# klasmodin/quflow

Measured on AMD Instinct MI355X. Metric: isospectral timesteps/sec at N=1024 (1 GPU) + ensemble steps/sec at 1/2/4/8 GPUs, higher is better.
Workload: dtype f64

## Files before the change

### include/quflow_hip.h

```cpp
#ifndef QUFLOW_HIP_H
#define QUFLOW_HIP_H

#ifdef __cplusplus
extern "C" {
#endif

#define QF_OK 0
#define QF_ERR_INVALID 1
#define QF_ERR_NO_DEVICE 2
#define QF_ERR_HIP 3
#define QF_ERR_STATE 4
#define QF_ERR_CALLBACK 5
#define QF_ERR_UNSUPPORTED 6
#define QF_ERR_NONFINITE 7
#define QF_ERR_NOCONVERGE 8

#define QF_VERSION 100

typedef struct qf_ctx qf_ctx;

int qf_version(void);
const char *qf_last_error(void);
int qf_device_count(void);

// ... 83 lines not shown
    int (*forcing)(void *user, const void *P, const void *Whalf, void *F, double time);
    int (*strang)(void *user, double h, void *W);
    int (*callback)(void *user, const void *W, const void *dW2);
    int hamiltonian_takes_time, forcing_takes_time;
    int has_time;
    double time;
    int skewh;
    int solve_skewh;
    const double *strang_table;
    unsigned long long strang_key;
    int magnetic;
    int states_p;
} qf_isomp_hooks;
int qf_isomp_hooked(qf_ctx *ctx, void *states_host, int k, double dt, int steps, double tol, int minit, int maxit,
                    int compsum, int reinitialize, const qf_isomp_hooks *hooks, qf_isomp_stats *stats_out);
int qf_isomp_forced(qf_ctx *ctx, double dt, int steps, double tol, int minit, int maxit, int reinitialize,
                    const double *strang_table, unsigned long long strang_key, qf_isomp_stats *stats_out);
int qf_erk_hooked(qf_ctx *ctx, void *W_host, int method, double dt, int steps, const qf_isomp_hooks *hooks);
int qf_erk_states_hooked(qf_ctx *ctx, void *states_host, int k, int method, double dt, int steps, const qf_isomp_hooks *hooks);

int qf_basis_upload(qf_ctx *ctx, const double *basis_host, long long count);
int qf_basis_compute(qf_ctx *ctx);
int qf_basis_download(qf_ctx *ctx, double *basis_host, long long count);
int qf_basis_stream(qf_ctx *ctx, long long slab_bytes);
int qf_basis_slab_plan(int N, int Nmax, long long slab_bytes, int *first_block, int capacity);
int qf_shr2mat(qf_ctx *ctx, const double *omega_host, long long n_omega, void *W_host);
int qf_mat2shr(qf_ctx *ctx, const void *W_host, double *omega_host, long long n_omega);
int qf_shc2mat(qf_ctx *ctx, const void *omega_host, void *W_host);
int qf_mat2shc(qf_ctx *ctx, const void *W_host, void *omega_host);
int qf_shr2fun(qf_ctx *ctx, const double *omega_host, long long n_omega, int L, int berezin, double *f_host);
int qf_shc2fun(qf_ctx *ctx, const void *omega_host, long long n_omega, int L, int berezin, int isreal, void *f_host);
int qf_fun2shc(qf_ctx *ctx, const void *f_host, int L, int isreal, void *omega_host);
int qf_fun2shr(qf_ctx *ctx, const void *f_host, int L, int isreal, double *omega_host);

int qf_diagnostics(qf_ctx *ctx, double *energy_euler, double *enstrophy);
int qf_isomp_diag(qf_ctx *ctx, double dt, int steps, double tol, int minit, int maxit, int compsum,
                  int reinitialize, qf_isomp_stats *stats, double *energy_euler, double *enstrophy);
int qf_norm_inf_W(qf_ctx *ctx, double *out);

typedef struct qf_eigh_stats {
    int sweeps;
    long long rotations;
    double off;
} qf_eigh_stats;
int qf_eigh(qf_ctx *ctx, const void *H_host, double *lambda_host, void *V_host, qf_eigh_stats *stats);
int qf_eigh_skew(qf_ctx *ctx, const void *W_host, double *lambda_host, void *V_host, qf_eigh_stats *stats);
int qf_eigh_state(qf_ctx *ctx, double *lambda_host, qf_eigh_stats *stats);
int qf_scale_decomposition(qf_ctx *ctx, const void *W_host, const void *P_host, void *Ws_host, void *Wr_host);

int qf_so3_exp_plan(int N, const double xi[3], int *squarings, int *degree);
int qf_so3_exp(qf_ctx *ctx, const double xi[3], void *R_host);
int qf_so3_exp_times(qf_ctx *ctx, double *taylor_ms, double *squarings_ms);
int qf_rotate(qf_ctx *ctx, const double xi[3], const void *W_host, void *out_host);
int qf_grad(qf_ctx *ctx, const void *P_host, void *dP_host);

#define QF_KERNEL_POISSON 0
#define QF_KERNEL_GEMM1 1
#define QF_KERNEL_GEMM2 2
#define QF_KERNEL_NORM 3
#define QF_KERNEL_UPDATE 4
#define QF_KERNEL_SLICE 5
#define QF_KERNEL_COUNT 6

int qf_profile_enable(qf_ctx *ctx, int mask);
int qf_profile_reset(qf_ctx *ctx);
int qf_profile_read(qf_ctx *ctx, int kernel_id, long long *launches, double *total_ms);
int qf_profile_stride(qf_ctx *ctx, int stride);
int qf_profile_seen(qf_ctx *ctx, int kernel_id, long long *seen);
int qf_device_info(int device, char *buf, int n);
int qf_plan_describe(qf_ctx *ctx, char *buf, int n);
int qf_timer_start(qf_ctx *ctx);
int qf_timer_stop(qf_ctx *ctx, double *elapsed_ms);

#define QF_BUF_W 0
#define QF_BUF_DW 1
#define QF_BUF_WHALF 2
#define QF_BUF_PHALF 3
#define QF_BUF_PW 4
int qf_download_buffer(qf_ctx *ctx, int which, void *host);
int qf_debug_guard_check(long long *allocations, long long *damaged, char *first, int n);
int qf_debug_modulus(qf_ctx *ctx, int n, const double *er_host, const double *ei_host, double *out_modulus_host,
                     double *out_sqrt_host);
int qf_zgemm(qf_ctx *ctx, const void *A_host, const void *B_host, void *C_host);
int qf_commutator(qf_ctx *ctx, const void *W_host, const void *P_host, void *C_host, int skewherm);
int qf_zgemm_i8(qf_ctx *ctx, const void *A_host, const void *B_host, void *C_host);
int qf_fixedpoint_products(qf_ctx *ctx, const void *Phalf_host, const void *Whalf_host, const void *W_host,
                           const void *dW_old_host, int variant, void *dW_new_host, void *Whalf_new_host,
                           double *rowsum_host);

int qf_c64_laplacian_table(qf_ctx *ctx, int bc, float *lap_host);
int qf_c64_solve_poisson(qf_ctx *ctx, const void *W_host, void *P_host, int skewh);
int qf_c64_solve_tridiagonal(qf_ctx *ctx, const float *lap_host, const void *W_host, void *P_host, int skewh);
int qf_c64_laplace(qf_ctx *ctx, const void *P_host, void *W_host);
int qf_c64_upload_W(qf_ctx *ctx, const void *W_host);
int qf_c64_download_W(qf_ctx *ctx, void *W_host);
int qf_c64_isomp(qf_ctx *ctx, double dt, int steps, double tol, int minit, int maxit, int compsum, int reinitialize,
                 qf_isomp_stats *stats_out);
int qf_c64_isomp_continue(qf_ctx *ctx, double dt, int steps, double tol, int minit, int maxit, int compsum, int reinitialize,
                          qf_isomp_stats *stats_out);
int qf_c64_diagnostics(qf_ctx *ctx, double *energy_euler, double *enstrophy);
int qf_cgemm(qf_ctx *ctx, const void *A_host, const void *B_host, void *C_host);
int qf_c64_fixedpoint_products(qf_ctx *ctx, const void *Phalf_host, const void *Whalf_host, const void *W_host,
                               const void *dW_old_host, void *dW_new_host, void *Whalf_new_host, double *rowsum_host);
int qf_c64_fixedpoint_products_tri(qf_ctx *ctx, const void *Phalf_host, const void *Whalf_host, const void *W_host,
                                   const void *dW_old_host, void *dW_new_host, void *Whalf_new_host, double *rowsum_host);

#define QF_COMM_ID_BYTES 128
typedef struct qf_comm qf_comm;
int qf_comm_unique_id(void *id128);
int qf_comm_create(qf_comm **out, int device, int nranks, int rank, const void *id128);
int qf_comm_allgather_f64(qf_comm *comm, const double *send_host, int count, double *recv_host);
int qf_comm_barrier(qf_comm *comm);
int qf_comm_destroy(qf_comm *comm);

#ifdef __cplusplus
}
#endif
#endif
```

### quflow_amd/_lib.py

```python
import ctypes
import os

_HERE = os.path.dirname(os.path.abspath(__file__))
LIB_PATH = os.environ.get("QUFLOW_HIP_LIB") or os.path.join(_HERE, "libquflow_hip.so")

QF_OK = 0
QF_ERR_NONFINITE = 7
QF_ERR_NOCONVERGE = 8
ERR_NAMES = {1: "QF_ERR_INVALID", 2: "QF_ERR_NO_DEVICE", 3: "QF_ERR_HIP", 4: "QF_ERR_STATE", 5: "QF_ERR_CALLBACK",
             6: "QF_ERR_UNSUPPORTED", 7: "QF_ERR_NONFINITE", 8: "QF_ERR_NOCONVERGE"}

KERNEL_IDS = {"poisson": 0, "gemm1": 1, "gemm2": 2, "norm": 3, "update": 4, "slice": 5}
ERK_METHODS = {"euler": 0, "heun": 1, "rk4": 2}
BUFFER_IDS = {"W": 0, "dW": 1, "Whalf": 2, "Phalf": 3, "PW": 4}


class QuflowHipError(RuntimeError):
    pass


HAMILTONIAN_CB = ctypes.CFUNCTYPE(ctypes.c_int, ctypes.c_void_p, ctypes.c_void_p, ctypes.c_void_p, ctypes.c_double)
FORCING_CB = ctypes.CFUNCTYPE(ctypes.c_int, ctypes.c_void_p, ctypes.c_void_p, ctypes.c_void_p, ctypes.c_void_p, ctypes.c_double)
STRANG_CB = ctypes.CFUNCTYPE(ctypes.c_int, ctypes.c_void_p, ctypes.c_double, ctypes.c_void_p)
CALLBACK_CB = ctypes.CFUNCTYPE(ctypes.c_int, ctypes.c_void_p, ctypes.c_void_p, ctypes.c_void_p)
# ... 63 lines not shown
    "qf_comm_unique_id": (ctypes.c_int, [_vp]),
    "qf_comm_create": (ctypes.c_int, [ctypes.POINTER(_vp), ctypes.c_int, ctypes.c_int, ctypes.c_int, _vp]),
    "qf_comm_allgather_f64": (ctypes.c_int, [_vp, _vp, ctypes.c_int, _vp]),
    "qf_comm_barrier": (ctypes.c_int, [_vp]),
    "qf_comm_destroy": (ctypes.c_int, [_vp]),
    "qf_upload_W": (ctypes.c_int, [_vp, _vp]),
    "qf_download_W": (ctypes.c_int, [_vp, _vp]),
    "qf_isomp": (ctypes.c_int, [_vp, ctypes.c_double, ctypes.c_int, ctypes.c_double, ctypes.c_int,
                                ctypes.c_int, ctypes.c_int, ctypes.c_int, ctypes.POINTER(IsompStats)]),
    "qf_isomp_diag": (ctypes.c_int, [_vp, ctypes.c_double, ctypes.c_int, ctypes.c_double, ctypes.c_int,
                                     ctypes.c_int, ctypes.c_int, ctypes.c_int, ctypes.POINTER(IsompStats),
                                     ctypes.POINTER(ctypes.c_double), ctypes.POINTER(ctypes.c_double)]),
    "qf_isomp_continue": (ctypes.c_int, [_vp, ctypes.c_double, ctypes.c_int, ctypes.c_double, ctypes.c_int,
                                         ctypes.c_int, ctypes.c_int, ctypes.c_int, ctypes.POINTER(IsompStats)]),
    "qf_isomp_multi": (ctypes.c_int, [ctypes.POINTER(_vp), ctypes.c_int, ctypes.c_double, ctypes.c_int, ctypes.c_double,
                                      ctypes.c_int, ctypes.c_int, ctypes.POINTER(IsompStats)]),
    "qf_c64_isomp_multi": (ctypes.c_int, [ctypes.POINTER(_vp), ctypes.c_int, ctypes.c_double, ctypes.c_int, ctypes.c_double,
                                          ctypes.c_int, ctypes.c_int, ctypes.POINTER(IsompStats)]),
    "qf_erk": (ctypes.c_int, [_vp, ctypes.c_int, ctypes.c_double, ctypes.c_int, ctypes.c_int]),
    "qf_erk_states": (ctypes.c_int, [_vp, _vp, ctypes.c_int, ctypes.c_int, ctypes.c_double, ctypes.c_int, ctypes.c_int]),
    "qf_isomp_simple_hooked": (ctypes.c_int, [_vp, ctypes.c_double, ctypes.c_int, ctypes.POINTER(IsompHooks)]),
    "qf_isomp_quasinewton_hooked": (ctypes.c_int, [_vp, ctypes.c_double, ctypes.c_int, ctypes.c_double, ctypes.c_int,
                                                   ctypes.POINTER(IsompStats), ctypes.POINTER(IsompHooks)]),
    "qf_isomp_simple": (ctypes.c_int, [_vp, ctypes.c_double, ctypes.c_int]),
    "qf_isomp_quasinewton": (ctypes.c_int, [_vp, ctypes.c_double, ctypes.c_int, ctypes.c_double, ctypes.c_int,
                                            ctypes.POINTER(IsompStats)]),
    "qf_isomp_states": (ctypes.c_int, [_vp, _vp, ctypes.c_int, ctypes.c_double, ctypes.c_int, ctypes.c_double,
                                       ctypes.c_int, ctypes.c_int, ctypes.c_int, ctypes.c_int,
                                       ctypes.POINTER(IsompStats)]),
    "qf_states_upload": (ctypes.c_int, [_vp, _vp, ctypes.c_int]),
    "qf_states_download": (ctypes.c_int, [_vp, _vp, ctypes.c_int]),
    "qf_states_advance": (ctypes.c_int, [_vp, ctypes.c_double, ctypes.c_int, ctypes.c_double, ctypes.c_int, ctypes.c_int,
                                         ctypes.c_int, ctypes.c_int, ctypes.POINTER(IsompStats)]),
    "qf_states_advance_diag": (ctypes.c_int, [_vp, ctypes.c_double, ctypes.c_int, ctypes.c_double, ctypes.c_int, ctypes.c_int,
                                              ctypes.c_int, ctypes.c_int, ctypes.POINTER(IsompStats), _dp]),
    "qf_states_select": (ctypes.c_int, [_vp, ctypes.c_int]),
    "qf_states_store": (ctypes.c_int, [_vp, ctypes.c_int]),
    "qf_mhd_diagnostics": (ctypes.c_int, [_vp, _dp]),
    "qf_states_inner": (ctypes.c_int, [_vp, _dp]),
    "qf_isomp_hooked": (ctypes.c_int, [_vp, _vp, ctypes.c_int, ctypes.c_double, ctypes.c_int, ctypes.c_double, ctypes.c_int,
                                       ctypes.c_int, ctypes.c_int, ctypes.c_int, ctypes.POINTER(IsompHooks),
                                       ctypes.POINTER(IsompStats)]),
    "qf_erk_hooked": (ctypes.c_int, [_vp, _vp, ctypes.c_int, ctypes.c_double, ctypes.c_int, ctypes.POINTER(IsompHooks)]),
    "qf_erk_states_hooked": (ctypes.c_int, [_vp, _vp, ctypes.c_int, ctypes.c_int, ctypes.c_double, ctypes.c_int,
                                            ctypes.POINTER(IsompHooks)]),
    "qf_basis_upload": (ctypes.c_int, [_vp, _vp, ctypes.c_longlong]),
    "qf_basis_compute": (ctypes.c_int, [_vp]),
    "qf_basis_download": (ctypes.c_int, [_vp, _vp, ctypes.c_longlong]),
    "qf_basis_stream": (ctypes.c_int, [_vp, ctypes.c_longlong]),
    "qf_basis_slab_plan": (ctypes.c_int, [ctypes.c_int, ctypes.c_int, ctypes.c_longlong, ctypes.POINTER(ctypes.c_int),
                                          ctypes.c_int]),
    "qf_shr2mat": (ctypes.c_int, [_vp, _vp, ctypes.c_longlong, _vp]),
    "qf_mat2shr": (ctypes.c_int, [_vp, _vp, _vp, ctypes.c_longlong]),
    "qf_shc2mat": (ctypes.c_int, [_vp, _vp, _vp]),
    "qf_mat2shc": (ctypes.c_int, [_vp, _vp, _vp]),
    "qf_shr2fun": (ctypes.c_int, [_vp, _vp, ctypes.c_longlong, ctypes.c_int, ctypes.c_int, _vp]),
    "qf_shc2fun": (ctypes.c_int, [_vp, _vp, ctypes.c_longlong, ctypes.c_int, ctypes.c_int, ctypes.c_int, _vp]),
    "qf_fun2shc": (ctypes.c_int, [_vp, _vp, ctypes.c_int, ctypes.c_int, _vp]),
    "qf_fun2shr": (ctypes.c_int, [_vp, _vp, ctypes.c_int, ctypes.c_int, _vp]),
    "qf_diagnostics": (ctypes.c_int, [_vp, _dp, _dp]),
    "qf_norm_inf_W": (ctypes.c_int, [_vp, _dp]),
    "qf_eigh": (ctypes.c_int, [_vp, _vp, _vp, _vp, ctypes.POINTER(EighStats)]),
    "qf_eigh_skew": (ctypes.c_int, [_vp, _vp, _vp, _vp, ctypes.POINTER(EighStats)]),
    "qf_eigh_state": (ctypes.c_int, [_vp, _vp, ctypes.POINTER(EighStats)]),
    "qf_scale_decomposition": (ctypes.c_int, [_vp, _vp, _vp, _vp, _vp]),
    "qf_so3_exp_plan": (ctypes.c_int, [ctypes.c_int, _dp, ctypes.POINTER(ctypes.c_int), ctypes.POINTER(ctypes.c_int)]),
    "qf_so3_exp": (ctypes.c_int, [_vp, _dp, _vp]),
    "qf_so3_exp_times": (ctypes.c_int, [_vp, _dp, _dp]),
    "qf_rotate": (ctypes.c_int, [_vp, _dp, _vp, _vp]),
    "qf_grad": (ctypes.c_int, [_vp, _vp, _vp]),
    "qf_profile_enable": (ctypes.c_int, [_vp, ctypes.c_int]),
    "qf_profile_reset": (ctypes.c_int, [_vp]),
    "qf_profile_read": (ctypes.c_int, [_vp, ctypes.c_int, ctypes.POINTER(ctypes.c_longlong), _dp]),
    "qf_plan_describe": (ctypes.c_int, [_vp, ctypes.c_char_p, ctypes.c_int]),
    "qf_device_info": (ctypes.c_int, [ctypes.c_int, ctypes.c_char_p, ctypes.c_int]),
    "qf_debug_modulus": (ctypes.c_int, [_vp, ctypes.c_int, _dp, _dp, _dp, _dp]),
    "qf_profile_stride": (ctypes.c_int, [_vp, ctypes.c_int]),
    "qf_profile_seen": (ctypes.c_int, [_vp, ctypes.c_int, ctypes.POINTER(ctypes.c_longlong)]),
    "qf_timer_start": (ctypes.c_int, [_vp]),
    "qf_timer_stop": (ctypes.c_int, [_vp, _dp]),
    "qf_download_buffer": (ctypes.c_int, [_vp, ctypes.c_int, _vp]),
    "qf_debug_guard_check": (ctypes.c_int, [ctypes.POINTER(ctypes.c_longlong), ctypes.POINTER(ctypes.c_longlong), ctypes.c_char_p, ctypes.c_int]),
    "qf_zgemm": (ctypes.c_int, [_vp, _vp, _vp, _vp]),
    "qf_commutator": (ctypes.c_int, [_vp, _vp, _vp, _vp, ctypes.c_int]),
    "qf_zgemm_i8": (ctypes.c_int, [_vp, _vp, _vp, _vp]),
    "qf_fixedpoint_products": (ctypes.c_int, [_vp, _vp, _vp, _vp, _vp, ctypes.c_int, _vp, _vp, _vp]),
    "qf_c64_laplacian_table": (ctypes.c_int, [_vp, ctypes.c_int, _vp]),
    "qf_c64_solve_poisson": (ctypes.c_int, [_vp, _vp, _vp, ctypes.c_int]),
    "qf_c64_laplace": (ctypes.c_int, [_vp, _vp, _vp]),
    "qf_c64_solve_tridiagonal": (ctypes.c_int, [_vp, _vp, _vp, _vp, ctypes.c_int]),
    "qf_c64_upload_W": (ctypes.c_int, [_vp, _vp]),
    "qf_c64_download_W": (ctypes.c_int, [_vp, _vp]),
    "qf_c64_isomp": (ctypes.c_int, [_vp, ctypes.c_double, ctypes.c_int, ctypes.c_double, ctypes.c_int,
                                    ctypes.c_int, ctypes.c_int, ctypes.c_int, ctypes.POINTER(IsompStats)]),
    "qf_c64_isomp_continue": (ctypes.c_int, [_vp, ctypes.c_double, ctypes.c_int, ctypes.c_double, ctypes.c_int,
                                             ctypes.c_int, ctypes.c_int, ctypes.c_int, ctypes.POINTER(IsompStats)]),
    "qf_c64_diagnostics": (ctypes.c_int, [_vp, _dp, _dp]),
    "qf_cgemm": (ctypes.c_int, [_vp, _vp, _vp, _vp]),
    "qf_c64_fixedpoint_products": (ctypes.c_int, [_vp, _vp, _vp, _vp, _vp, _vp, _vp, _vp]),
    "qf_c64_fixedpoint_products_tri": (ctypes.c_int, [_vp, _vp, _vp, _vp, _vp, _vp, _vp, _vp]),
}

_lib = None


def load():
    global _lib
    if _lib is None:
        if not os.path.exists(LIB_PATH):
            raise QuflowHipError(
                "libquflow_hip.so is not built (%s). Run `python -c 'import __graft_entry__ as g; g.build()'` "
                "or `make -C quflow_amd/csrc`. There is no CPU fallback." % LIB_PATH)
        lib = ctypes.CDLL(LIB_PATH)
        for name, (res, args) in SIGNATURES.items():
            fn = getattr(lib, name)
            fn.restype = res
            fn.argtypes = args
        _lib = lib
    return _lib


def check(rc):
    if rc == 7:
        raise ValueError("array must not contain infs or NaNs")
    if rc != QF_OK:
        msg = load().qf_last_error()
        raise QuflowHipError("%s: %s" % (ERR_NAMES.get(rc, "error %d" % rc),
                                         msg.decode("utf-8", "replace") if msg else ""))


def check_eigh(rc):
    if rc != QF_OK:
        msg = load().qf_last_error()
        raise QuflowHipError("%s: %s" % (ERR_NAMES.get(rc, "error %d" % rc),
                                         msg.decode("utf-8", "replace") if msg else ""))


def device_count():
    return load().qf_device_count()


def device_info(device):
    import json
    lib = load()
    n = lib.qf_device_info(int(device), None, 0)
    if n < 0:
        check(-n)
    buf = ctypes.create_string_buffer(n + 1)
    lib.qf_device_info(int(device), buf, n + 1)
    return json.loads(buf.value.decode())
```

### quflow_amd/csrc/api_context.hip

```cpp
#include <cmath>
#include <cstdarg>
#include <cstdio>
#include <cstdlib>
#include <cstring>
#include <limits>
#include <chrono>

#include "qf_api.h"

static thread_local char g_err[512] = "";

void qf_set_error(const char *fmt, ...)
{
    va_list ap;
    va_start(ap, fmt);
    vsnprintf(g_err, sizeof(g_err), fmt, ap);
    va_end(ap);
}

extern "C" {

int qf_version(void) { return QF_VERSION; }

int qf_device_info(int device, char *buf, int n)
// ... 33 lines not shown
    if (!ctx || (n > 0 && !buf) || n < 0) {
        qf_set_error("qf_plan_describe: bad arguments");
        return -QF_ERR_INVALID;
    }
    static const char *const role[QF_KERNEL_COUNT] = {"laplacian_inverse", "first_product", "second_product", "residual_norm",
                                                      "step_update", "slicing"};
    std::string out = "{\"N\": " + std::to_string(ctx->N);
    for (int r = 0; r < QF_KERNEL_COUNT; ++r) {
        out += ", \"";
        out += role[r];
        out += "\": ";
        out += ctx->plan[r].text[0] ? ctx->plan[r].text : "null";
    }
    if (ctx->ham_table || ctx->ham_offset_on) {
        char h[160];
        if (ctx->ham_table) snprintf(h, sizeof(h), ", \"hamiltonian\": {\"table_key\": %llu, \"offset\": %s}", ctx->ham_key, ctx->ham_offset_on ? "true" : "false");
        else snprintf(h, sizeof(h), ", \"hamiltonian\": {\"table_key\": null, \"offset\": true}");
        out += h;
    } else {
        out += ", \"hamiltonian\": \"poisson\"";
    }
    out += "}";
    if (n > 0) {
        const size_t m = out.size() < (size_t)(n - 1) ? out.size() : (size_t)(n - 1);
        memcpy(buf, out.data(), m);
        buf[m] = 0;
    }
    return (int)out.size();
}

const char *qf_last_error(void) { return g_err; }

int qf_device_count(void)
{
    int n = 0;
    if (hipGetDeviceCount(&n) != hipSuccess) return 0;
    return n;
}

double qf_hbar(int N) { return 2.0 / std::sqrt((double)N * (double)N - 1.0); }

int qf_ctx_create(int N, int device, qf_ctx **out)
{
    if (!out) {
        qf_set_error("qf_ctx_create: out is null");
        return QF_ERR_INVALID;
    }
    *out = nullptr;
    if (N < 2 || N > 8192) {
        qf_set_error("qf_ctx_create: N=%d out of range [2, 8192]", N);
        return QF_ERR_INVALID;
    }
    int ndev = qf_device_count();
    if (ndev <= 0) {
        qf_set_error("qf_ctx_create: no HIP device visible (this library has no CPU fallback)");
        return QF_ERR_NO_DEVICE;
    }
    if (device < 0 || device >= ndev) {
        qf_set_error("qf_ctx_create: device %d out of range (0..%d)", device, ndev - 1);
        return QF_ERR_NO_DEVICE;
    }
    QF_HIP(hipSetDevice(device));
    qf_ctx *ctx = new qf_ctx();
    ctx->N = N;
    ctx->device = device;
    if (const char *g = getenv("QUFLOW_HIP_GEMM")) {
        ctx->gemm_i8_allowed = (g[0] == 'i');
        if (g[0] == 'i' && strstr(g, "x6")) ctx->oz_digits = 6;
        if (g[0] == 'i' && strstr(g, "x65")) ctx->oz_digits2 = 5;
        if (g[0] == 'i' && strchr(g, 'h')) ctx->gemm_i8_hybrid = true;
        if (g[0] == 'i' && strchr(g, 'f') && !ctx->gemm_i8_hybrid) ctx->gemm_i8_first = true;
        if (g[0] == 'a') {
            ctx->gemm_i8_allowed = true;
            ctx->oz_digits = 6;
            ctx->oz_digits2 = 5;
            ctx->gemm_i8_min_n = 1024;
        }
    }
    if (const char *g = getenv("QUFLOW_HIP_GEMM2")) ctx->gemm_tri_allowed = !(g[0] == 'f');
    if (const char *g = getenv("QUFLOW_HIP_FUSED")) ctx->fused_allowed = !(g[0] == '0');
    if (const char *g = getenv("QUFLOW_HIP_I8_MIN_N")) ctx->gemm_i8_min_n = atoi(g);
    if (const char *g = getenv("QUFLOW_HIP_TRI_MIN_N")) ctx->gemm_tri_min_n = atoi(g);
    if (const char *g = getenv("QUFLOW_HIP_DEFER")) ctx->defer_allowed = !(g[0] == '0');
    if (getenv("QUFLOW_HIP_DEBUG"))
        if (const char *g = getenv("QUFLOW_HIP_DEBUG_DROP_FLAG")) ctx->debug_drop = atoi(g);
    if (const char *g = getenv("QUFLOW_HIP_FACTOR_CACHE_MB")) ctx->factor_budget_bytes = (size_t)(atoi(g) > 0 ? atoi(g) : 1) << 20;
    const size_t NN = (size_t)N * N;
    const size_t mbytes = NN * sizeof(cplx);
    int rc = QF_OK;
    auto fail = [&](int code) {
        qf_ctx_destroy(ctx);
        return code;
    };
#define QF_CREATE_HIP(call)                                                                   \
    do {                                                                                      \
        hipError_t _e = (call);                                                               \
        if (_e != hipSuccess) {                                                               \
            qf_set_error("%s failed: %s", #call, hipGetErrorString(_e));                     \
            return fail(QF_ERR_HIP);                                                          \
        }                                                                                     \
    } while (0)
    QF_CREATE_HIP(hipStreamCreateWithFlags(&ctx->stream, hipStreamNonBlocking));
    cplx **mats[] = {&ctx->W, &ctx->dW[0], &ctx->dW[1], &ctx->Whalf, &ctx->Phalf, &ctx->PW, &ctx->stage};
    for (cplx **m : mats) {
        QF_CREATE_HIP(hipMalloc((void **)m, mbytes));
        QF_CREATE_HIP(hipMemsetAsync(*m, 0, mbytes, ctx->stream));
    }
    QF_CREATE_HIP(hipMalloc((void **)&ctx->lap, 2 * NN * sizeof(double)));
    ctx->rowpart_tiles = qf_gemm_tiles_n(N);
    {
        const int slots32 = (N + 31) / 32;
        QF_CREATE_HIP(hipMalloc((void **)&ctx->rowpart, (size_t)(ctx->rowpart_tiles > slots32 ? ctx->rowpart_tiles : slots32) * N * sizeof(double)));
    }
    QF_CREATE_HIP(hipMalloc((void **)&ctx->rowsum, (size_t)N * sizeof(double)));
    QF_CREATE_HIP(hipMalloc((void **)&ctx->scalars, 4096 * sizeof(double)));
    QF_CREATE_HIP(hipHostMalloc((void **)&ctx->host_scalars, 64 * sizeof(double), hipHostMallocDefault));
    QF_CREATE_HIP(hipMalloc((void **)&ctx->state, sizeof(qf_dev_state)));
    QF_CREATE_HIP(hipMemsetAsync(ctx->state, 0, sizeof(qf_dev_state), ctx->stream));
    QF_CREATE_HIP(hipMalloc((void **)&ctx->ticket, 704 * sizeof(unsigned)));
    QF_CREATE_HIP(hipMemsetAsync(ctx->ticket, 0, 704 * sizeof(unsigned), ctx->stream));
    QF_CREATE_HIP(hipHostMalloc((void **)&ctx->host_rec, sizeof(qf_host_record), hipHostMallocCoherent));
    memset(ctx->host_rec, 0, sizeof(qf_host_record));
    {
        hipDeviceProp_t prop;
        QF_CREATE_HIP(hipGetDeviceProperties(&prop, device));
        ctx->num_cus = prop.multiProcessorCount;
        if (N % 64 == 0 && ctx->num_cus > 0) {
            ctx->sk_slots = ctx->num_cus;
            QF_CREATE_HIP(hipMalloc((void **)&ctx->sk_partial, (size_t)ctx->sk_slots * 64 * 64 * sizeof(cplx)));
            QF_CREATE_HIP(hipMalloc((void **)&ctx->sk_flags, (size_t)(ctx->sk_slots + 16) * sizeof(unsigned)));
            QF_CREATE_HIP(hipMemsetAsync(ctx->sk_flags, 0, (size_t)(ctx->sk_slots + 16) * sizeof(unsigned), ctx->stream));
        }
    }
    QF_CREATE_HIP(hipEventCreate(&ctx->timer_start));
    QF_CREATE_HIP(hipEventCreate(&ctx->timer_stop));
#undef QF_CREATE_HIP
    if ((rc = alloc_factors(ctx, &ctx->poisson)) != QF_OK) return fail(rc);
    if ((rc = qf_launch_lap_table(ctx, 1, ctx->lap)) != QF_OK) return fail(rc);
    if ((rc = qf_launch_build_factors(ctx, ctx->lap, ctx->poisson)) != QF_OK) return fail(rc);
    if (hipStreamSynchronize(ctx->stream) != hipSuccess) {
        qf_set_error("qf_ctx_create: table construction failed");
        return fail(QF_ERR_HIP);
    }
    *out = ctx;
    return QF_OK;
}

int qf_ctx_destroy(qf_ctx *ctx)
{
    if (!ctx) return QF_OK;
    (void)hipSetDevice(ctx->device);
    if (ctx->stream) (void)hipStreamSynchronize(ctx->stream);
    void *ptrs[] = {ctx->W, ctx->dW[0], ctx->dW[1], ctx->Whalf, ctx->Phalf, ctx->PW, ctx->kahan_c, ctx->stage,
                    ctx->lap, ctx->lap_user, ctx->poisson.tab, ctx->ham.tab, ctx->ham_offset, ctx->forcing_f0, ctx->stoch.basis, ctx->stoch.omega,
                    ctx->stoch.stage, ctx->stoch.sigma, ctx->rowpart, ctx->rowsum,
                    ctx->t32_partial, ctx->t32_arrive, ctx->W2, ctx->Whalf2, ctx->ns_inv, ctx->ns_tmp, ctx->multi_rowpart, ctx->scalars, ctx->sk_partial, ctx->sk_flags, ctx->basis, ctx->sh_stage, ctx->sh_omega, ctx->slab};
    for (void *p : ptrs)
        if (p) (void)hipFree(p);
    void *sht[] = {ctx->sht.omega, ctx->sht.tab, ctx->sht.col, ctx->sht.At, ctx->sht.tw, ctx->sht.f, ctx->sht.H, ctx->sht.Q};
    for (void *p : sht)
        if (p) (void)hipFree(p);
    void *eigh[] = {ctx->eigh.H, ctx->eigh.G, ctx->eigh.V, ctx->eigh.ray, ctx->eigh.sig, ctx->eigh.perm, ctx->eigh.word};
    for (void *p : eigh)
        if (p) (void)hipFree(p);
    void *geom[] = {ctx->geom.R[0], ctx->geom.R[1], ctx->geom.grad};
    for (void *p : geom)
// ... 228 lines not shown
```

### quflow_amd/csrc/api_isomp.hip

```cpp
#include <cmath>
#include <cstdarg>
#include <cstdio>
#include <cstdlib>
#include <cstring>
#include <limits>
#include <chrono>
#include <type_traits>
#include <utility>

#include "qf_api.h"

namespace {

#ifndef QF_RUN_AHEAD
#define QF_RUN_AHEAD 3
#endif

template <class S> constexpr bool is_c64 = std::is_same<S, qf_c64>::value;

template <class S> S *ws(qf_ctx *ctx)
{
    if constexpr (is_c64<S>) return ctx->c64;
    else return ctx;
}
// ... 99 lines not shown
        if (f->w_skew_known) {
            QF_TRY(qf_c64_tri_alloc(ctx));
            f->tri = true;
        }
    }
    return QF_OK;
}

bool triangle_product(const qf_ctx *ctx) { return (ctx->gemm_tri || ctx->gemm_tri32) && (!ctx->gemm_i8 || ctx->gemm_i8_first); }
bool triangle_product(const qf_c64 *f) { return f->tri; }

template <class S> int begin_increment(qf_ctx *ctx, S *w, bool carry)
{
    const size_t mbytes = (size_t)ctx->N * ctx->N * sizeof(*w->W);
    if (carry) {
        if (w->dw_cur != 0)
            QF_HIP(hipMemcpyAsync(w->dW[0], w->dW[w->dw_cur], mbytes, hipMemcpyDeviceToDevice, ctx->stream));
        QF_TRY(qf_launch_lincomb(ctx, 1, w->W, 1, w->dW[0], 0, w->Whalf));
    } else {
        QF_HIP(hipMemsetAsync(w->dW[0], 0, mbytes, ctx->stream));
        QF_HIP(hipMemcpyAsync(w->Whalf, w->W, mbytes, hipMemcpyDeviceToDevice, ctx->stream));
    }
    return QF_OK;
}

template <class S> int enqueue_iterations(qf_ctx *ctx, int step, int first, int count, double vareps)
{
    S *w = ws<S>(ctx);
    for (int i = first; i < first + count; ++i) {
        qf_guard g;
        g.state = ctx->state;
        g.step = step;
        g.iter = i;
        {
            prof_scope p(ctx, QF_KERNEL_POISSON);
            QF_TRY(launch_solve(ctx, w->Whalf, w->Phalf, vareps, g));
        }
        {
            prof_scope p(ctx, QF_KERNEL_GEMM1);
            QF_TRY(launch_gemm(ctx, w->Phalf, w->Whalf, w->PW, nullptr, g));
        }
        {
            prof_scope p(ctx, QF_KERNEL_GEMM2);
            const auto ep = epilogue_of(w, false);
            QF_TRY(launch_gemm(ctx, w->PW, w->Phalf, nullptr, &ep, g));
        }
        {
            prof_scope p(ctx, QF_KERNEL_NORM);
            QF_TRY(qf_launch_norm_decide(ctx, w->rowpart, is_c64<S> ? w->rowpart_tiles : qf_rowpart_slots(ctx), g));
        }
    }
    return QF_OK;
}

qf_decide deferred_decision(qf_ctx *ctx)
{
    qf_decide d;
    d.rowpart = ctx->rowpart;
    d.slots = ctx->gemm_tri32 ? (ctx->N + 31) / 32 : ctx->N / 64;
    d.state_rw = ctx->state;
    d.rec = ctx->host_rec;
    d.ticket = ctx->ticket + 402;
    return d;
}

template <class S> int enqueue_iterations_fused(qf_ctx *ctx, int step, int first, int count, double vareps, bool last_step)
{
    S *w = ws<S>(ctx);
    const bool defer = !is_c64<S> && ctx->defer;
    const qf_decide dec = defer ? deferred_decision(ctx) : qf_decide();
    for (int i = first; i < first + count; ++i) {
        qf_guard g;
        g.state = ctx->state;
        g.step = step;
        g.iter = i;
        g.alt = w->Whalf2;
        {
            prof_scope p(ctx, QF_KERNEL_POISSON);
            if constexpr (is_c64<S>) QF_TRY(launch_solve(ctx, w->Whalf, w->Phalf, vareps, g));
            else QF_TRY(launch_solve(ctx, w->Whalf, w->Phalf, vareps, g, defer ? &dec : nullptr));
        }
        {
            prof_scope p(ctx, QF_KERNEL_GEMM1);
            QF_TRY(launch_gemm(ctx, w->Phalf, w->Whalf, w->PW, nullptr, g));
        }
        {
            prof_scope p(ctx, QF_KERNEL_GEMM2);
            const auto ep = epilogue_of(w, true);
            g.alt = nullptr;
            if constexpr (is_c64<S>) {
                if (w->tri) QF_TRY(qf_launch_cgemm_tri(ctx, w->PW, w->Phalf, &ep, g));
                else QF_TRY(qf_launch_cgemm(ctx, w->PW, w->Phalf, nullptr, &ep, g));
            } else {
                QF_TRY(qf_launch_zgemm(ctx, w->PW, w->Phalf, nullptr, &ep, g));
            }
        }
    }
    if (defer && last_step && count > 0) QF_TRY(qf_launch_decide(ctx, dec));
    return QF_OK;
}

int enqueue_iterations_fused_i8(qf_ctx *ctx, int step, int first, int count, double vareps)
{
    for (int i = first; i < first + count; ++i) {
        qf_guard g;
        g.state = ctx->state;
        g.step = step;
        g.iter = i;
        g.alt = ctx->Whalf2;
        {
            prof_scope p(ctx, QF_KERNEL_POISSON);
            QF_TRY(qf_launch_hamiltonian(ctx, ctx->Whalf, ctx->Phalf, vareps, g));
        }
        if (ctx->gemm_i8_hybrid) {
            {
                prof_scope p(ctx, QF_KERNEL_GEMM1);
                QF_TRY(qf_launch_zgemm(ctx, ctx->Phalf, ctx->Whalf, ctx->PW, nullptr, g));
            }
            g.alt = nullptr;
            {
                prof_scope p(ctx, QF_KERNEL_SLICE);
                qf_oz_jobs jobs;
                jobs.n = 2;
                jobs.j[0].X = ctx->PW;
                jobs.j[0].planes = ctx->oz_planes[3];
                jobs.j[0].scale = ctx->oz_scale[3];
                jobs.j[1].X = ctx->Phalf;
                jobs.j[1].planes = ctx->oz_planes[0];
                jobs.j[1].scale = ctx->oz_scale[0];
                QF_TRY(qf_launch_oz_slice(ctx, jobs, g));
            }
            {
                prof_scope p(ctx, QF_KERNEL_GEMM2);
                const qf_epilogue ep = epilogue_of(ctx, true);
                QF_TRY(qf_launch_oz_gemm(ctx, ctx->oz_planes[3], ctx->oz_scale[3], ctx->oz_planes[0], ctx->oz_scale[0], nullptr,
                                         &ep, g));
            }
            continue;
        }
        g.alt = nullptr;
        {
            prof_scope p(ctx, QF_KERNEL_SLICE);
            qf_oz_jobs jobs;
            jobs.n = 2;
            jobs.j[0].X = ctx->Phalf;
            jobs.j[0].planes = ctx->oz_planes[0];
            jobs.j[0].scale = ctx->oz_scale[0];
            jobs.j[1].X = ctx->Whalf;
            jobs.j[1].X_alt = ctx->Whalf2;
            jobs.j[1].planes = ctx->oz_planes[2];
            jobs.j[1].scale = ctx->oz_scale[2];
            jobs.diag = ctx->oz_diag;
            QF_TRY(qf_launch_oz_slice(ctx, jobs, g));
        }
        {
            prof_scope p(ctx, QF_KERNEL_GEMM1);
            QF_TRY(qf_launch_oz_gemm(ctx, ctx->oz_planes[0], ctx->oz_scale[0], ctx->oz_planes[2], ctx->oz_scale[2],
                                     ctx->PW, nullptr, g, 0, 0, ctx->oz_diag));
        }
        if (ctx->gemm_i8_first) {
            prof_scope p(ctx, QF_KERNEL_GEMM2);
            const qf_epilogue ep = epilogue_of(ctx, true);
            QF_TRY(qf_launch_zgemm(ctx, ctx->PW, ctx->Phalf, nullptr, &ep, g));
            continue;
        }
        {
            prof_scope p(ctx, QF_KERNEL_SLICE);
            qf_oz_jobs jobs;
            jobs.n = 1;
            jobs.j[0].X = ctx->PW;
            jobs.j[0].planes = ctx->oz_planes[3];
// ... 126 lines not shown
        sched_yield();
        return;
    }
#if defined(__x86_64__)
    __builtin_ia32_pause();
#endif
}

template <class S> int run_fused(qf_ctx *ctx, int steps, int minit, int maxit, double vareps)
{
    fused_run<S> run;
    run.begin(ctx, steps, minit, maxit, vareps);
    while (!run.done()) {
        QF_TRY(run.pump());
        poll_relax();
    }
    ctx->pred_iters = run.pred;
    return QF_OK;
}

template <class S> int enqueue_step_end(qf_ctx *ctx, int step, int compsum, int reinitialize)
{
    S *w = ws<S>(ctx);
    qf_guard g;
    g.state = ctx->state;
    g.step = step;
    prof_scope p(ctx, QF_KERNEL_UPDATE);
    return qf_launch_update(ctx, w->PW, w->W, w->dW[0], w->dW[1], w->Whalf, compsum ? w->kahan_c : nullptr, reinitialize, g);
}

int wait_for_advance(qf_ctx *ctx, unsigned long long seq)
{
    volatile qf_host_record *rec = ctx->host_rec;
    unsigned long long spins = 0;
    while (__atomic_load_n(&rec->seq, __ATOMIC_ACQUIRE) < seq) {
        if (++spins > (1ull << 22)) {
            const unsigned long long before = __atomic_load_n(&rec->seq, __ATOMIC_ACQUIRE);
            const hipError_t q = hipStreamQuery(ctx->stream);
            QF_HIP(hipStreamSynchronize(ctx->stream));
            if (getenv("QUFLOW_HIP_DEBUG"))
                fprintf(stderr, "[quflow_hip] wait_for_advance: spin limit; want seq %llu, saw %llu before sync (stream %s), %llu after; step_index %d incomplete %d\n",
                        seq, before, q == hipSuccess ? "idle" : "busy", (unsigned long long)rec->seq, rec->step_index, rec->incomplete);
            if (__atomic_load_n(&rec->seq, __ATOMIC_ACQUIRE) < seq) {
                qf_set_error("qf_isomp: device progress record stuck at %llu (< %llu)",
                             (unsigned long long)rec->seq, seq);
                return QF_ERR_STATE;
            }
            break;
        }
#if defined(__x86_64__)
        __builtin_ia32_pause();
#endif
    }
    return QF_OK;
}

int reset_after_abort(qf_ctx *ctx)
{
    if (!ctx->needs_reset) return QF_OK;
    QF_HIP(hipMemsetAsync(ctx->ticket, 0, 704 * sizeof(unsigned), ctx->stream));
    if (ctx->sk_flags) QF_HIP(hipMemsetAsync(ctx->sk_flags + (ctx->sk_slots > 0 ? ctx->sk_slots : ctx->num_cus), 0, 16 * sizeof(unsigned), ctx->stream));
    if (ctx->t32_arrive) {
        const size_t nt = (size_t)(ctx->N + 31) / 32;
        QF_HIP(hipMemsetAsync(ctx->t32_arrive, 0, nt * (nt + 1) / 2 * sizeof(unsigned), ctx->stream));
    }
    if (ctx->c64 && ctx->c64->tri_arrive)
        QF_HIP(hipMemsetAsync(ctx->c64->tri_arrive, 0, ctx->c64->tri_arrive_count * sizeof(unsigned), ctx->stream));
    ctx->needs_reset = false;
    return QF_OK;
}

template <class S> int fused_enter(qf_ctx *ctx, double dt, double tol, int minit, int maxit, bool carry)
{
    S *w = ws<S>(ctx);
    const size_t mbytes = (size_t)ctx->N * ctx->N * sizeof(*w->W);
    const bool tol_on_device = tol < 0;
    const double tol_factor = tol_on_device ? mach_eps<S>(true) * dt / qf_hbar(ctx->N) : 0.0;
    QF_TRY(reset_after_abort(ctx));
    if constexpr (is_c64<S>) {
        QF_TRY(select_second_product_c64(ctx));
    } else {
        QF_TRY(select_second_product(ctx));
        ctx->defer = ctx->defer_allowed && !ctx->gemm_i8 && ctx->gemm_tri32 && ctx->N <= 512;
    }
    w->increment_is_zero = !carry;
    w->increment_valid = true;
    volatile qf_host_record *rec = ctx->host_rec;
    rec->progress = 0ull;
    rec->step_index = 0;
    rec->fault = 0;
    rec->nonfinite = 0;
    __atomic_thread_fence(__ATOMIC_SEQ_CST);
    if (is_c64<S> || carry) {
        if (tol_on_device) QF_TRY(qf_launch_norm_inf(ctx, w->W, ctx->scalars));
        QF_TRY(begin_increment(ctx, w, carry));
        QF_TRY(qf_launch_state_init(ctx, tol, minit, maxit, tol_on_device ? ctx->scalars : nullptr, tol_factor));
    } else {
        QF_TRY(qf_launch_call_begin(ctx, tol, minit, maxit, tol_on_device ? 1 : 0, tol_factor));
    }
    if (!w->W2) QF_HIP(hipMalloc((void **)&w->W2, mbytes));
    if (!w->Whalf2) QF_HIP(hipMalloc((void **)&w->Whalf2, mbytes));
    if constexpr (!is_c64<S>)
        if (ctx->gemm_i8) QF_TRY(qf_oz_alloc(ctx));
    return QF_OK;
}

template <class S> int fused_leave(qf_ctx *ctx, int steps, qf_isomp_stats *stats_out)
{
    S *w = ws<S>(ctx);
    volatile qf_host_record *rec = ctx->host_rec;
    const int w_parity = steps > 0 ? rec->w_parity : 0, wh_sel = steps > 0 ? rec->wh_sel : 0;
    w->dw_cur = steps > 0 ? rec->dw_parity : 0;
    if (w_parity) std::swap(w->W, w->W2);
    if (wh_sel) std::swap(w->Whalf, w->Whalf2);
    if (triangle_product(w) && steps > 0) {
        QF_TRY(qf_launch_mirror_lower(ctx, w->W));
        QF_TRY(qf_launch_mirror_lower(ctx, w->dW[w->dw_cur]));
    }
    if constexpr (!is_c64<S>)
        if (ctx->diag_at_exit) {
            QF_TRY(qf_enqueue_diagnostics(ctx));
            ctx->diag_valid = true;
        }
    QF_HIP(hipStreamSynchronize(ctx->stream));
    if (rec->nonfinite) {
        qf_set_error("array must not contain infs or NaNs");
        ctx->needs_reset = true;
        w->increment_valid = false;
        ctx->diag_valid = false;
        rec->nonfinite = 0;
        return QF_ERR_NONFINITE;
    }
    if (steps > 0 && rec->step_index != steps) {
        qf_set_error("qf_isomp: device completed %d of %d steps (internal error)", rec->step_index, steps);
        return QF_ERR_STATE;
    }
    if (rec->fault) {
        qf_set_error("qf_isomp: a device-side wait of the second product ran out (a parked partial tile or a mirrored result tile was never published)");
        return QF_ERR_STATE;
    }
    if (stats_out) {
        stats_out->total_iterations = steps > 0 ? rec->total_iterations : 0;
        stats_out->number_of_maxit = steps > 0 ? rec->number_of_maxit : 0;
        stats_out->tol_used = rec->tol;
        stats_out->last_resnorm = rec->resnorm;
    }
    return QF_OK;
}

void fused_abort(qf_ctx *ctx)
{
    (void)hipStreamSynchronize(ctx->stream);
    ctx->needs_reset = true;
    ctx->increment_valid = false;
    ctx->w_skew_known = false;
    if (ctx->c64) {
        ctx->c64->w_skew_known = false;
        ctx->c64->increment_valid = false;
    }
    ctx->host_rec->fault = 0;
    ctx->host_rec->nonfinite = 0;
}

template <class S>
int isomp_impl(qf_ctx *ctx, double dt, int steps, double tol, int minit, int maxit, int compsum, int reinitialize,
               qf_isomp_stats *stats_out, bool carry_increment)
{
    QF_TRY(check_ctx(ctx));
    if (minit < 1) {
        qf_set_error("minit must be at least 1.");
        return QF_ERR_INVALID;
    }
    if (maxit < minit) {
        qf_set_error("maxit must be at minit.");
        return QF_ERR_INVALID;
    }
    if (steps < 0) {
        qf_set_error("qf_isomp: steps must be >= 0");
        return QF_ERR_INVALID;
    }
    QF_TRY(qf_refuse_forcing(ctx, is_c64<S> ? "qf_c64_isomp" : "qf_isomp"));
    const bool dbg = getenv("QUFLOW_HIP_DEBUG") != nullptr;
    auto now = [] { return std::chrono::steady_clock::now(); };
    auto ms_since = [&](std::chrono::steady_clock::time_point t) {
        return std::chrono::duration<double, std::milli>(now() - t).count();
    };
    const auto t_entry = now();
    double t_tol = 0, t_sel = 0, t_init = 0, t_loop = 0, t_waitmax = 0, t_waitat = 0, t_enqmax = 0, t_enqat = 0;
    int waitstep = -1, enqstep = -1;
    S *w = ws<S>(ctx);
    const int N = ctx->N;
    const size_t mbytes = (size_t)N * N * sizeof(*w->W);
    const double hb = qf_hbar(N);
    const double vareps = dt / (2 * hb);
    const bool carry = carry_increment && w->increment_valid && !reinitialize;

    if (ctx->fused_allowed && !compsum && !reinitialize) {
        int rc = fused_enter<S>(ctx, dt, tol, minit, maxit, carry);
        t_init = ms_since(t_entry);
        if (rc == QF_OK) rc = run_fused<S>(ctx, steps, minit, maxit, vareps);
        const double t_run = ms_since(t_entry);
// ... 222 lines not shown
    QF_HIP(hipMemcpyAsync(f->Whalf, Whalf_host, bytes, hipMemcpyHostToDevice, ctx->stream));
    QF_HIP(hipMemcpyAsync(f->stage, W_host, bytes, hipMemcpyHostToDevice, ctx->stream));
    QF_HIP(hipMemcpyAsync(f->dW[0], dW_old_host, bytes, hipMemcpyHostToDevice, ctx->stream));
    QF_TRY(qf_launch_cgemm(ctx, f->Phalf, f->Whalf, f->PW, nullptr));
    qf_epilogue_f ep = epilogue_of(f, false);
    ep.W = f->stage;
    if (tri) {
        QF_TRY(qf_launch_cgemm_tri(ctx, f->PW, f->Phalf, &ep));
        QF_TRY(qf_launch_mirror_lower(ctx, f->dW[1]));
        QF_TRY(qf_launch_sum_rowpart(ctx, f->rowpart, (N + qf_c64_tile(ctx) - 1) / qf_c64_tile(ctx), ctx->rowsum));
    } else {
        QF_TRY(qf_launch_cgemm(ctx, f->PW, f->Phalf, nullptr, &ep));
        QF_TRY(qf_launch_sum_rowpart(ctx, f->rowpart, f->rowpart_tiles, ctx->rowsum));
    }
    QF_HIP(hipMemcpyAsync(dW_new_host, f->dW[1], bytes, hipMemcpyDeviceToHost, ctx->stream));
    QF_HIP(hipMemcpyAsync(Whalf_new_host, f->Whalf, bytes, hipMemcpyDeviceToHost, ctx->stream));
    QF_HIP(hipMemcpyAsync(rowsum_host, ctx->rowsum, (size_t)N * sizeof(double), hipMemcpyDeviceToHost, ctx->stream));
    QF_HIP(hipStreamSynchronize(ctx->stream));
    return QF_OK;
}

}

int qf_rowpart_slots(const qf_ctx *ctx) { return ctx->gemm_tri ? ctx->N / 64 : ctx->gemm_tri32 ? (ctx->N + 31) / 32 : ctx->rowpart_tiles; }

int qf_enqueue_diagnostics(qf_ctx *ctx)
{
    QF_TRY(qf_launch_solve(ctx, ctx->poisson, ctx->W, ctx->stage, 1.0, 1));
    QF_TRY(qf_launch_inner2(ctx, ctx->W, ctx->stage, ctx->scalars + 2));
    QF_HIP(hipMemcpyAsync(ctx->host_scalars, ctx->scalars + 2, 2 * sizeof(double), hipMemcpyDeviceToHost, ctx->stream));
    return QF_OK;
}

int qf_isomp_multi(qf_ctx **ctxs, int k, double dt, int steps, double tol, int minit, int maxit, qf_isomp_stats *stats_out)
{
    return isomp_multi<qf_ctx>(ctxs, k, dt, steps, tol, minit, maxit, stats_out);
}

int qf_c64_isomp_multi(qf_ctx **ctxs, int k, double dt, int steps, double tol, int minit, int maxit, qf_isomp_stats *stats_out)
{
    return isomp_multi<qf_c64>(ctxs, k, dt, steps, tol, minit, maxit, stats_out);
}

int qf_isomp(qf_ctx *ctx, double dt, int steps, double tol, int minit, int maxit, int compsum,
             int reinitialize, qf_isomp_stats *stats_out)
{
    return isomp_impl<qf_ctx>(ctx, dt, steps, tol, minit, maxit, compsum, reinitialize, stats_out, false);
}

int qf_isomp_continue(qf_ctx *ctx, double dt, int steps, double tol, int minit, int maxit, int compsum,
                      int reinitialize, qf_isomp_stats *stats_out)
{
    return isomp_impl<qf_ctx>(ctx, dt, steps, tol, minit, maxit, compsum, reinitialize, stats_out, true);
}

int qf_isomp_diag(qf_ctx *ctx, double dt, int steps, double tol, int minit, int maxit, int compsum, int reinitialize,
                  qf_isomp_stats *stats_out, double *energy_euler, double *enstrophy)
{
    QF_TRY(check_ctx(ctx));
    ctx->diag_at_exit = true;
    ctx->diag_valid = false;
    const int rc = isomp_impl<qf_ctx>(ctx, dt, steps, tol, minit, maxit, compsum, reinitialize, stats_out, false);
    ctx->diag_at_exit = false;
    if (rc != QF_OK) return rc;
    if (!ctx->diag_valid) return qf_diagnostics(ctx, energy_euler, enstrophy);
    ctx->diag_valid = false;
    const double wp = ctx->host_scalars[0], ww = ctx->host_scalars[1];
    if (energy_euler) *energy_euler = -(wp / ctx->N) / 2.0;
    if (enstrophy) *enstrophy = (ww / ctx->N) / 2.0;
    return QF_OK;
}


int qf_fixedpoint_products(qf_ctx *ctx, const void *Phalf_host, const void *Whalf_host, const void *W_host,
                           const void *dW_old_host, int variant, void *dW_new_host, void *Whalf_new_host,
                           double *rowsum_host)
{
    QF_TRY(check_ctx(ctx));
    if (!Phalf_host || !Whalf_host || !W_host || !dW_old_host || !dW_new_host || !Whalf_new_host || !rowsum_host) {
        qf_set_error("qf_fixedpoint_products: null buffer");
        return QF_ERR_INVALID;
    }
    const int variant_arg = variant;
    variant &= 15;
    if (variant == 1 && !ctx->sk_partial) {
        qf_set_error("qf_fixedpoint_products: the upper-triangle product needs N %% 64 == 0 (N=%d)", ctx->N);
        return QF_ERR_INVALID;
    }
    if (variant == 2) {
        if (ctx->N < 64) {
            qf_set_error("qf_fixedpoint_products: the 32x32 upper-triangle product needs N >= 64 (N=%d)", ctx->N);
            return QF_ERR_INVALID;
        }
        QF_TRY(tri32_alloc(ctx));
    }
    const int N = ctx->N;
    const size_t bytes = (size_t)N * N * sizeof(cplx);
    QF_HIP(hipMemcpyAsync(ctx->Phalf, Phalf_host, bytes, hipMemcpyHostToDevice, ctx->stream));
    QF_HIP(hipMemcpyAsync(ctx->Whalf, Whalf_host, bytes, hipMemcpyHostToDevice, ctx->stream));
    QF_HIP(hipMemcpyAsync(ctx->stage, W_host, bytes, hipMemcpyHostToDevice, ctx->stream));
    QF_HIP(hipMemcpyAsync(ctx->dW[0], dW_old_host, bytes, hipMemcpyHostToDevice, ctx->stream));
    QF_TRY(qf_launch_zgemm(ctx, ctx->Phalf, ctx->Whalf, ctx->PW, nullptr));
    qf_epilogue ep = epilogue_of(ctx, false);
    ep.W = ctx->stage;
    const bool saved = ctx->gemm_tri, saved32 = ctx->gemm_tri32;
    const int s_min = ctx->sk_min_units, s_epi = ctx->sk_epi_units, s_so = ctx->tri32_split, s_sd = ctx->tri32_split_diag;
    ctx->gemm_tri = (variant == 1);
    ctx->gemm_tri32 = (variant == 2);
    if (variant == 1) {
        if ((variant_arg >> 8) & 0xff) ctx->sk_min_units = (variant_arg >> 8) & 0xff;
        if ((variant_arg >> 16) & 0xff) ctx->sk_epi_units = ((variant_arg >> 16) & 0xff) - 64;
    } else if (variant == 2) {
        const int so = (variant_arg >> 8) & 15, sd = (variant_arg >> 12) & 15;
        if (so == 1 || so == 2 || so == 4) ctx->tri32_split = so;
        if (sd == 1 || sd == 2 || sd == 4) ctx->tri32_split_diag = sd;
    }
    int rc = qf_launch_zgemm(ctx, ctx->PW, ctx->Phalf, nullptr, &ep);
    ctx->gemm_tri = saved;
    ctx->gemm_tri32 = saved32;
    ctx->sk_min_units = s_min;
    ctx->sk_epi_units = s_epi;
    ctx->tri32_split = s_so;
    ctx->tri32_split_diag = s_sd;
    QF_TRY(rc);
    QF_TRY(qf_launch_sum_rowpart(ctx, ctx->rowpart, variant == 1 ? ctx->N / 64 : variant == 2 ? (ctx->N + 31) / 32 : ctx->rowpart_tiles, ctx->rowsum));
    QF_HIP(hipMemcpyAsync(dW_new_host, ctx->dW[1], bytes, hipMemcpyDeviceToHost, ctx->stream));
    QF_HIP(hipMemcpyAsync(Whalf_new_host, ctx->Whalf, bytes, hipMemcpyDeviceToHost, ctx->stream));
    QF_HIP(hipMemcpyAsync(rowsum_host, ctx->rowsum, (size_t)N * sizeof(double), hipMemcpyDeviceToHost, ctx->stream));
    QF_HIP(hipStreamSynchronize(ctx->stream));
    return QF_OK;
}


int qf_oz_alloc(qf_ctx *ctx)
{
    for (int q = 0; q < 4; ++q) {
        if (!ctx->oz_planes[q]) QF_HIP(hipMalloc((void **)&ctx->oz_planes[q], qf_oz_operand_bytes(ctx->N, ctx->oz_digits)));
        if (!ctx->oz_scale[q])
            QF_HIP(hipMalloc((void **)&ctx->oz_scale[q], qf_oz_record_bytes(ctx->N, ctx->oz_digits)));
    }
    if (!ctx->oz_diag) QF_HIP(hipMalloc((void **)&ctx->oz_diag, (size_t)ctx->N * sizeof(double)));
    if (!ctx->oz_tbuf) {
        const size_t t = (size_t)(ctx->N / 64), nup = t * (t + 1) / 2;
        QF_HIP(hipMalloc((void **)&ctx->oz_tbuf, nup * 64 * 64 * sizeof(cplx)));
        QF_HIP(hipMalloc((void **)&ctx->oz_tflags, nup * sizeof(unsigned)));
        QF_HIP(hipMemsetAsync(ctx->oz_tflags, 0, nup * sizeof(unsigned), ctx->stream));
    }
    return QF_OK;
}


int qf_c64_isomp(qf_ctx *ctx, double dt, int steps, double tol, int minit, int maxit, int compsum, int reinitialize,
                 qf_isomp_stats *stats_out)
{
    QF_TRY(qf_need_c64(ctx));
    return isomp_impl<qf_c64>(ctx, dt, steps, tol, minit, maxit, compsum, reinitialize, stats_out, false);
}

int qf_c64_isomp_continue(qf_ctx *ctx, double dt, int steps, double tol, int minit, int maxit, int compsum, int reinitialize,
                          qf_isomp_stats *stats_out)
{
    QF_TRY(qf_need_c64(ctx));
    return isomp_impl<qf_c64>(ctx, dt, steps, tol, minit, maxit, compsum, reinitialize, stats_out, true);
}

int qf_c64_fixedpoint_products(qf_ctx *ctx, const void *Phalf_host, const void *Whalf_host, const void *W_host,
                               const void *dW_old_host, void *dW_new_host, void *Whalf_new_host, double *rowsum_host)
{
    return c64_fixedpoint_products("qf_c64_fixedpoint_products", false, ctx, Phalf_host, Whalf_host, W_host, dW_old_host,
                                   dW_new_host, Whalf_new_host, rowsum_host);
}

int qf_c64_fixedpoint_products_tri(qf_ctx *ctx, const void *Phalf_host, const void *Whalf_host, const void *W_host,
                                   const void *dW_old_host, void *dW_new_host, void *Whalf_new_host, double *rowsum_host)
{
    return c64_fixedpoint_products("qf_c64_fixedpoint_products_tri", true, ctx, Phalf_host, Whalf_host, W_host, dW_old_host,
                                   dW_new_host, Whalf_new_host, rowsum_host);
}
```

### quflow_amd/csrc/api_transforms.hip

```cpp
#include <cmath>
#include <cstdarg>
#include <cstdio>
#include <cstdlib>
#include <cstring>
#include <limits>
#include <chrono>
#include <algorithm>
#include <vector>

#include "qf_api.h"

extern "C" {

static int need_basis(qf_ctx *ctx, const char *who)
{
    if (!ctx->basis) {
        qf_set_error("%s: no quantization basis on this context (call qf_basis_upload first)", who);
        return QF_ERR_STATE;
    }
    return QF_OK;
}

static int alloc_stage(qf_ctx *ctx);

// ... 309 lines not shown
    const size_t LL = (size_t)L * L;
    QF_HIP(hipMemcpyAsync(ctx->sht.f, f_host, (size_t)L * (2 * (size_t)L - 1) * (isreal ? sizeof(double) : sizeof(cplx)),
                          hipMemcpyHostToDevice, ctx->stream));
    if (!out_dev) out_dev = ctx->sht.omega;
    QF_TRY(qf_launch_sht_analysis(ctx, L, shr, isreal, out_dev));
    if (omega_host)
        QF_HIP(hipMemcpyAsync(omega_host, out_dev, LL * (shr ? sizeof(double) : sizeof(cplx)), hipMemcpyDeviceToHost, ctx->stream));
    QF_HIP(hipStreamSynchronize(ctx->stream));
    return QF_OK;
}

int qf_fun2shc(qf_ctx *ctx, const void *f_host, int L, int isreal, void *omega_host)
{
    QF_TRY(check_ctx(ctx));
    if (!omega_host) {
        qf_set_error("qf_fun2shc: null coefficient array");
        return QF_ERR_INVALID;
    }
    return sht_analyse(ctx, "qf_fun2shc", f_host, L, isreal ? 1 : 0, 0, nullptr, omega_host);
}

int qf_fun2shr(qf_ctx *ctx, const void *f_host, int L, int isreal, double *omega_host)
{
    QF_TRY(check_ctx(ctx));
    if (omega_host) return sht_analyse(ctx, "qf_fun2shr", f_host, L, isreal ? 1 : 0, 1, nullptr, omega_host);
    if (L > ctx->N) {
        qf_set_error("qf_fun2shr: omega == NULL keeps L^2 coefficients on a context of N^2: L=%d exceeds N=%d", L, ctx->N);
        return QF_ERR_INVALID;
    }
    QF_TRY(alloc_stage(ctx));
    ctx->sh_shr_count = 0;
    QF_TRY(sht_analyse(ctx, "qf_fun2shr", f_host, L, isreal ? 1 : 0, 1, ctx->sh_omega, nullptr));
    ctx->sh_shr_count = (long long)L * L;
    return QF_OK;
}


int qf_zgemm_i8(qf_ctx *ctx, const void *A_host, const void *B_host, void *C_host)
{
    QF_TRY(check_ctx(ctx));
    if (!A_host || !B_host || !C_host) {
        qf_set_error("qf_zgemm_i8: null buffer");
        return QF_ERR_INVALID;
    }
    if (ctx->N % 64 != 0) {
        qf_set_error("qf_zgemm_i8: N=%d is not a multiple of 64", ctx->N);
        return QF_ERR_INVALID;
    }
    QF_TRY(qf_oz_alloc(ctx));
    const size_t bytes = (size_t)ctx->N * ctx->N * sizeof(cplx);
    QF_HIP(hipMemcpyAsync(ctx->stage, A_host, bytes, hipMemcpyHostToDevice, ctx->stream));
    QF_HIP(hipMemcpyAsync(ctx->Phalf, B_host, bytes, hipMemcpyHostToDevice, ctx->stream));
    qf_oz_jobs jobs;
    jobs.n = 2;
    jobs.j[0].X = ctx->stage;
    jobs.j[0].planes = ctx->oz_planes[0];
    jobs.j[0].scale = ctx->oz_scale[0];
    jobs.j[1].X = ctx->Phalf;
    jobs.j[1].planes = ctx->oz_planes[1];
    jobs.j[1].scale = ctx->oz_scale[1];
    QF_TRY(qf_launch_oz_slice(ctx, jobs));
    QF_TRY(qf_launch_oz_gemm(ctx, ctx->oz_planes[0], ctx->oz_scale[0], ctx->oz_planes[1], ctx->oz_scale[1], ctx->PW));
    QF_HIP(hipMemcpyAsync(C_host, ctx->PW, bytes, hipMemcpyDeviceToHost, ctx->stream));
    QF_HIP(hipStreamSynchronize(ctx->stream));
    return QF_OK;
}

int qf_zgemm(qf_ctx *ctx, const void *A_host, const void *B_host, void *C_host)
{
    QF_TRY(check_ctx(ctx));
    if (!A_host || !B_host || !C_host) {
        qf_set_error("qf_zgemm: null buffer");
        return QF_ERR_INVALID;
    }
    const size_t bytes = (size_t)ctx->N * ctx->N * sizeof(cplx);
    QF_HIP(hipMemcpyAsync(ctx->stage, A_host, bytes, hipMemcpyHostToDevice, ctx->stream));
    QF_HIP(hipMemcpyAsync(ctx->Phalf, B_host, bytes, hipMemcpyHostToDevice, ctx->stream));
    QF_TRY(qf_launch_zgemm(ctx, ctx->stage, ctx->Phalf, ctx->PW, nullptr));
    QF_HIP(hipMemcpyAsync(C_host, ctx->PW, bytes, hipMemcpyDeviceToHost, ctx->stream));
    QF_HIP(hipStreamSynchronize(ctx->stream));
    return QF_OK;
}

int qf_commutator(qf_ctx *ctx, const void *W_host, const void *P_host, void *C_host, int skewherm)
{
    QF_TRY(check_ctx(ctx));
    if (!W_host || !P_host || !C_host) {
        qf_set_error("qf_commutator: null buffer");
        return QF_ERR_INVALID;
    }
    const size_t bytes = (size_t)ctx->N * ctx->N * sizeof(cplx);
    QF_HIP(hipMemcpyAsync(ctx->stage, W_host, bytes, hipMemcpyHostToDevice, ctx->stream));
    QF_HIP(hipMemcpyAsync(ctx->Phalf, P_host, bytes, hipMemcpyHostToDevice, ctx->stream));
    QF_TRY(qf_launch_zgemm(ctx, ctx->stage, ctx->Phalf, ctx->PW, nullptr));
    if (skewherm) {
        QF_TRY(qf_launch_neg_conj_transpose(ctx, ctx->PW, ctx->Whalf));
        QF_TRY(qf_launch_lincomb(ctx, 1.0, ctx->PW, 1.0, ctx->Whalf, 0.0, ctx->PW));
    } else {
        QF_TRY(qf_launch_zgemm(ctx, ctx->Phalf, ctx->stage, ctx->Whalf, nullptr));
        QF_TRY(qf_launch_lincomb(ctx, 1.0, ctx->PW, -1.0, ctx->Whalf, 0.0, ctx->PW));
    }
    QF_HIP(hipMemcpyAsync(C_host, ctx->PW, bytes, hipMemcpyDeviceToHost, ctx->stream));
    QF_HIP(hipStreamSynchronize(ctx->stream));
    return QF_OK;
}


int qf_cgemm(qf_ctx *ctx, const void *A_host, const void *B_host, void *C_host)
{
    QF_TRY(qf_need_c64(ctx));
    if (!A_host || !B_host || !C_host) {
        qf_set_error("qf_cgemm: null buffer");
        return QF_ERR_INVALID;
    }
    qf_c64 *f = ctx->c64;
    const size_t bytes = (size_t)ctx->N * ctx->N * sizeof(float2);
    QF_HIP(hipMemcpyAsync(f->stage, A_host, bytes, hipMemcpyHostToDevice, ctx->stream));
    QF_HIP(hipMemcpyAsync(f->Phalf, B_host, bytes, hipMemcpyHostToDevice, ctx->stream));
    QF_TRY(qf_launch_cgemm(ctx, f->stage, f->Phalf, f->PW, nullptr));
    QF_HIP(hipMemcpyAsync(C_host, f->PW, bytes, hipMemcpyDeviceToHost, ctx->stream));
    QF_HIP(hipStreamSynchronize(ctx->stream));
    return QF_OK;
}


}
```

### quflow_amd/csrc/qf_internal.h

```cpp
#pragma once

#include <hip/hip_runtime.h>

#include <atomic>
#include <cstdarg>
#include <cstdio>
#include <map>
#include <mutex>
#include <string>
#include <vector>

#include "../../include/quflow_hip.h"

typedef double2 cplx;

hipError_t qf_guard_malloc(void **p, size_t bytes);
hipError_t qf_guard_free(void *p);
#define hipMalloc(p, n) qf_guard_malloc((void **)(p), (n))
#define hipFree(p) qf_guard_free((void *)(p))

void qf_set_error(const char *fmt, ...);
struct qf_ctx;
inline void qf_plan_note(qf_ctx *ctx, unsigned long long key, const char *fmt, ...) __attribute__((format(printf, 3, 4)));

#define QF_HIP(call)                                                                   \
    do {                                                                               \
        hipError_t _e = (call);                                                        \
        if (_e != hipSuccess) {                                                        \
            qf_set_error("%s failed: %s (%s:%d)", #call, hipGetErrorString(_e), __FILE__, __LINE__); \
            return QF_ERR_HIP;                                                         \
        }                                                                              \
    } while (0)

#define QF_TRY(call)              \
    do {                          \
        int _r = (call);          \
        if (_r != QF_OK) return _r; \
    } while (0)

struct qf_factors {
    double2 *tab = nullptr;
};

#define QF_FAULT_WAIT 1
#define QF_FAULT_NONFINITE 2
#define QF_STEP_ABORTED 0x40000000
#define QF_FINITE(x_) ((x_) <= 1.7976931348623157e308 && (x_) >= -1.7976931348623157e308)

struct qf_dev_state {
    double resnorm;
    double tol;
    long long total_iterations;
    long long number_of_maxit;
    int step_index;
    int iters_this_step;
    int step_done;
    int minit, maxit;
    int dw_parity;
    int fault;
    int w_parity;
    int wh_sel;
    int pending;
    int pending_iter;
};


struct qf_host_record {
    unsigned long long seq;
    long long total_iterations;
    long long number_of_maxit;
    double resnorm;
    int step_index;
    int last_step_iters;
    int incomplete;
    int nonfinite;
    unsigned long long progress;
    double tol;
    int w_parity, wh_sel, dw_parity;
    int fault;
};

struct qf_decide {
    const double *rowpart = nullptr;
    int slots = 0;
    qf_dev_state *state_rw = nullptr;
    qf_host_record *rec = nullptr;
    unsigned *ticket = nullptr;
};

struct qf_guard {
    const qf_dev_state *state = nullptr;
    int step = 0;
    int iter = 0;
    const void *alt = nullptr;
};

#ifdef __HIPCC__
__device__ __forceinline__ bool qf_guard_iter(const qf_guard &g)
{
    if (!g.state) return true;
    return g.state->step_index == g.step && g.state->step_done == 0 && g.state->iters_this_step == g.iter;
}
__device__ __forceinline__ bool qf_guard_step_end(const qf_guard &g)
{
    if (!g.state) return true;
    return g.state->step_index == g.step && (g.state->step_done != 0 || g.state->iters_this_step >= g.state->maxit);
}
template <int CTRL> __device__ __forceinline__ double qf_dpp_f64(double v)
{
    const int lo = __builtin_amdgcn_update_dpp(0, __double2loint(v), CTRL, 0xf, 0xf, true);
    const int hi = __builtin_amdgcn_update_dpp(0, __double2hiint(v), CTRL, 0xf, 0xf, true);
    return __hiloint2double(hi, lo);
}
__device__ __forceinline__ double qf_row16_sum(double v)
{
    v += qf_dpp_f64<0xB1>(v);
    v += qf_dpp_f64<0x4E>(v);
    v += qf_dpp_f64<0x141>(v);
    v += qf_dpp_f64<0x140>(v);
    return v;
}

__device__ __forceinline__ double qf_modulus(double er, double ei)
{
    const double x = er * er + ei * ei;
    const double y = __builtin_amdgcn_rsq(x);
    double g = x * y, h = 0.5 * y;
    const double r = __builtin_fma(-h, g, 0.5);
    g = __builtin_fma(g, r, g);
    h = __builtin_fma(h, r, h);
    double d = __builtin_fma(-g, g, x);
    g = __builtin_fma(d, h, g);
    d = __builtin_fma(-g, g, x);
    g = __builtin_fma(d, h, g);
    return (x > 0.0 && x < __builtin_inf()) ? g : x;
}

__device__ __forceinline__ double qf_lap_b(int N, int i, int j)
{
    long long k = i < j ? i : j;
    long long am = i < j ? j - i : i - j;
    long long NN = N;
    return -(double)((NN - 1) * (2 * k + 1 + am) - 2 * k * (k + am));
}
__device__ __forceinline__ double qf_lap_a(int N, int i, int j)
{
    long long k = i < j ? i : j;
    long long am = i < j ? j - i : i - j;
    long long NN = N;
    return sqrt((double)(((k + am) * (NN - k - am)) * (k * (NN - k))));
}
template <typename R, typename C2>
__device__ __forceinline__ C2 qf_laplace_entry(int N, const C2 *__restrict__ P, int i, int j)
{
#pragma clang fp contract(off)
    const size_t e = (size_t)i * N + j;
    R b = (R)qf_lap_b(N, i, j);
    C2 p = P[e];
    R wr = b * p.x, wi = b * p.y;
    if (i < N - 1 && j < N - 1) {
        R a = (R)qf_lap_a(N, i + 1, j + 1);
        C2 q = P[e + N + 1];
        wr += a * q.x;
        wi += a * q.y;
    }
    if (i > 0 && j > 0) {
        R a = (R)qf_lap_a(N, i, j);
        C2 q = P[e - N - 1];
        wr += a * q.x;
        wi += a * q.y;
    }
    C2 o;
    o.x = wr;
    o.y = wi;
    return o;
}
#endif
// ... 115 lines not shown
    bool w_skew_known = false;
    cplx *dW[2] = {nullptr, nullptr};
    int dw_cur = 0;
    bool increment_is_zero = true;
    int pred_first_iters = 0;
    bool increment_valid = false;
    cplx *W2 = nullptr;
    cplx *Whalf2 = nullptr;
    bool fused_allowed = true;
    cplx *Whalf = nullptr;
    cplx *Phalf = nullptr;
    cplx *PW = nullptr;
    cplx *kahan_c = nullptr;
    cplx *stage = nullptr;
    signed char *oz_planes[4] = {nullptr, nullptr, nullptr, nullptr};
    double *oz_scale[4] = {nullptr, nullptr, nullptr, nullptr};
    bool gemm_i8 = false;
    bool gemm_i8_allowed = false;
    bool gemm_i8_hybrid = false;
    bool gemm_i8_first = false;
    int gemm_i8_min_n = 768;
    int oz_digits = 5;
    int oz_digits2 = 0;
    cplx *oz_tbuf = nullptr;
    unsigned *oz_tflags = nullptr;
    unsigned oz_epoch = 0;
    double *oz_diag = nullptr;
    std::vector<cplx *> multi;
    double *multi_rowpart = nullptr;
    std::vector<cplx *> stack;
    int stack_k = 0;
    double *mhd_part = nullptr;
    cplx *hook_host[3] = {nullptr, nullptr, nullptr};
    size_t hook_host_bytes = 0;
    cplx *ns_inv = nullptr;
    cplx *ns_tmp = nullptr;

    double *lap = nullptr;
    qf_factors poisson;
    struct factor_entry {
        qf_factors f;
        unsigned long long fingerprint = 0;
        unsigned long long last_used = 0;
    };
    std::map<unsigned long long, factor_entry> user_factors;
    unsigned long long factor_clock = 0;
    size_t factor_budget_bytes = (size_t)512 << 20;
    double *lap_user = nullptr;
    qf_factors ham;
    unsigned long long ham_key = 0, ham_fp = 0;
    cplx *ham_offset = nullptr;
    unsigned long long ham_offset_key = 0, ham_offset_fp = 0;
    bool ham_table = false, ham_offset_on = false;
    cplx *forcing_f0 = nullptr;
    unsigned long long forcing_key = 0, forcing_fp = 0;
    bool forcing_on = false, forcing_f0_on = false;
    double forcing_aW = 0.0, forcing_aP = 0.0, forcing_alap = 0.0;
    qf_stoch stoch;

    double *basis = nullptr;
    cplx *sh_stage = nullptr;
    double *sh_omega = nullptr;
    long long sh_shr_count = 0;
    long long slab_budget = 0;
    double *slab = nullptr;
    size_t slab_cap = 0;
    qf_sht sht;
    qf_eigh_ws eigh;
    qf_geom_ws geom;

    double *rowpart = nullptr;
    int rowpart_tiles = 0;
    double *rowsum = nullptr;
    double *scalars = nullptr;
    double *host_scalars = nullptr;
    qf_dev_state *state = nullptr;
    qf_host_record *host_rec = nullptr;
    bool diag_at_exit = false, diag_valid = false;
    unsigned *ticket = nullptr;
    int pred_iters = 3;
    bool gemm_tri_allowed = true;
    bool gemm_tri = false;
    int gemm_tri_min_n = 960;
    bool gemm_tri32 = false;
    int tri32_split = 2, tri32_split_diag = 1;
    cplx *t32_partial = nullptr;
    unsigned *t32_arrive = nullptr;
    bool defer_allowed = true;
    bool defer = false;
    int num_cus = 0;
    cplx *sk_partial = nullptr;
    unsigned *sk_flags = nullptr;
    int sk_slots = 0;
    unsigned sk_epoch = 0;
    int sk_epi_units = 0;
    int sk_epi_units_fused = 2;
    int sk_min_units = 8;
    int debug_drop = 0;
    bool needs_reset = false;

    qf_c64 *c64 = nullptr;

    int profile_mask = 0;
    std::vector<qf_event_pair> events_busy;
    std::vector<qf_event_pair> events_free;
    int profile_stride = 1;
    struct plan_slot {
        unsigned long long key = 0;
        char text[384] = {0};
    } plan[QF_KERNEL_COUNT];
    int plan_role = -1;
    long long prof_seen[QF_KERNEL_COUNT] = {0};
    long long prof_launches[QF_KERNEL_COUNT] = {0};
    double prof_ms[QF_KERNEL_COUNT] = {0};
    hipEvent_t timer_start = nullptr, timer_stop = nullptr;
};

inline void qf_plan_note(qf_ctx *ctx, unsigned long long key, const char *fmt, ...)
{
    if (!ctx || ctx->plan_role < 0 || ctx->plan_role >= QF_KERNEL_COUNT) return;
    qf_ctx::plan_slot &s = ctx->plan[ctx->plan_role];
    if (key != 0 && s.key == key) return;
    va_list ap;
    va_start(ap, fmt);
    vsnprintf(s.text, sizeof(s.text), fmt, ap);
    va_end(ap);
    s.key = key;
}

inline int qf_refuse_forcing(const qf_ctx *ctx, const char *who)
{
    if (ctx && ctx->forcing_on) {
        qf_set_error("%s: a forcing is installed on this context (qf_set_forcing) and this entry point cannot apply it; "
                     "qf_isomp_forced, qf_isomp_hooked (k = 1) and qf_erk_hooked follow an installed forcing", who);
        return QF_ERR_UNSUPPORTED;
    }
    return QF_OK;
}

int qf_launch_forcing_affine(qf_ctx *ctx, const cplx *Ph, const cplx *X, cplx *out, double pscale, double s);

int qf_launch_stoch_pattern(qf_ctx *ctx, unsigned long long step, double dt);

int qf_launch_lap_table(qf_ctx *ctx, int bc, double *lap_dev);
int qf_launch_build_factors(qf_ctx *ctx, const double *lap_dev, qf_factors f);
int qf_launch_solve(qf_ctx *ctx, const qf_factors &f, const cplx *W, cplx *P, double scale, int skewh,
                    qf_guard guard = qf_guard(), const qf_decide *dec = nullptr);
int qf_launch_decide(qf_ctx *ctx, const qf_decide &dec);
int qf_launch_hamiltonian(qf_ctx *ctx, const cplx *W, cplx *P, double scale, qf_guard guard = qf_guard(),
                          const qf_decide *dec = nullptr);
int qf_launch_laplace(qf_ctx *ctx, const cplx *P, cplx *W);
int qf_launch_laplace_scaled(qf_ctx *ctx, const cplx *P, cplx *W, double scale);

int qf_launch_lap_table(qf_ctx *ctx, int bc, float *lap_dev);
int qf_launch_build_factors(qf_ctx *ctx, const float *lap_dev, float2 *tab);
int qf_launch_solve(qf_ctx *ctx, const float2 *tab, const float2 *W, float2 *P, float scale, int skewh,
                    qf_guard guard = qf_guard());
int qf_launch_laplace(qf_ctx *ctx, const float2 *P, float2 *W);

int qf_c64_alloc(qf_ctx *ctx);
void qf_c64_free(qf_c64 *f);
int qf_launch_cgemm(qf_ctx *ctx, const float2 *A, const float2 *B, float2 *C, const qf_epilogue_f *ep, qf_guard guard = qf_guard());
int qf_c64_tile(const qf_ctx *ctx);
int qf_c64_tile_first(const qf_ctx *ctx);
int qf_c64_tri_alloc(qf_ctx *ctx);
int qf_launch_cgemm_tri(qf_ctx *ctx, const float2 *A, const float2 *B, const qf_epilogue_f *ep, qf_guard guard = qf_guard());

struct qf_epilogue {
    const cplx *PW = nullptr;
    const cplx *W = nullptr;
    cplx *dW[2] = {nullptr, nullptr};
    cplx *Whalf = nullptr;
    double *rowpart = nullptr;
    int fused = 0;
    cplx *Wpair[2] = {nullptr, nullptr};
    cplx *Whalf_step = nullptr;
    unsigned *ticket = nullptr;
    int n_tiles = 0;
    qf_dev_state *state_rw = nullptr;
    qf_host_record *rec = nullptr;
    int debug_drop = 0;
};
struct qf_streamk {
    cplx *partial = nullptr;
    unsigned *flags = nullptr;
    unsigned epoch = 0;
    int *fault = nullptr;
    unsigned *ticket = nullptr;
    int n_tiles = 0;
    qf_dev_state *state_rw = nullptr;
    qf_host_record *rec = nullptr;
    unsigned spin_limit = 1u << 22;
    int debug_drop = 0;
    int slots = 0;
};
struct qf_tri32 {
    cplx *partial = nullptr;
    unsigned *arrive = nullptr;
    int split = 1;
    int split_diag = 1;
    unsigned *ticket = nullptr;
    int n_tiles = 0;
    qf_dev_state *state_rw = nullptr;
    qf_host_record *rec = nullptr;
    int debug_drop = 0;
    int deferred = 0;
};
int qf_gemm_tiles_n(int N);
int qf_launch_zgemm_tri32(qf_ctx *ctx, const cplx *A, const cplx *B, const qf_epilogue *ep, qf_guard guard = qf_guard());
int qf_launch_zgemm_tri(qf_ctx *ctx, const cplx *A, const cplx *B, const qf_epilogue *ep, qf_guard guard = qf_guard());
int qf_launch_zgemm(qf_ctx *ctx, const cplx *A, const cplx *B, cplx *C, const qf_epilogue *ep,
                    qf_guard guard = qf_guard());

int qf_launch_basis(qf_ctx *ctx, double *basis_dev);
__host__ __device__ inline long long qf_slab_prefix(int N, int Nmax, int m)
{
    const long long a = m, n = N, k = Nmax;
    return a * n * k - (n + k) * (a * (a - 1) / 2) + (a - 1) * a * (2 * a - 1) / 6;
}
int qf_slab_plan(int N, int Nmax, long long slab_bytes, std::vector<int> &first, long long *max_bytes);
int qf_launch_shr2mat(qf_ctx *ctx, int Nmax, const double *omega_dev, cplx *W_dev);
int qf_launch_band_basis(qf_ctx *ctx, int Nmax, double *band_dev);
int qf_launch_band_shr2mat(qf_ctx *ctx, int Nmax, const double *band_dev, const double *omega_dev, cplx *stage, cplx *W_dev);
int qf_launch_mat2shr(qf_ctx *ctx, int Nmax, const cplx *W_dev, double *omega_dev);
int qf_launch_shc2mat(qf_ctx *ctx, const double *omega_dev, cplx *W_dev);
int qf_launch_mat2shc(qf_ctx *ctx, const cplx *W_dev, double *omega_dev);

int qf_launch_sht_synth(qf_ctx *ctx, int L, int shr, int isreal, const double *omega_dev, long long n_valid);
void qf_sht_sizes(int L, int isreal, size_t bytes[6]);
int qf_launch_sht_analysis(qf_ctx *ctx, int L, int shr, int isreal, double *omega_dev);
int qf_launch_sht_qbuild(qf_ctx *ctx, int L);
void qf_sht_analysis_sizes(int L, int isreal, size_t bytes[8]);

int qf_launch_eigh_round(qf_ctx *ctx, cplx *G, int round, double tol, unsigned long long *word);
int qf_launch_eigh_normalise(qf_ctx *ctx, cplx *G, double *sig);
int qf_launch_eigh_rowdot(qf_ctx *ctx, const cplx *T, const cplx *U, cplx *out);
int qf_launch_eigh_conj_transpose(qf_ctx *ctx, const cplx *U, const int *perm, const cplx *scale, cplx *out);
int qf_launch_eigh_neg_i(qf_ctx *ctx, const cplx *X, cplx *out);

#define QF_SO3_STRIP 32
#define QF_SO3_MAX_DEGREE 16
int qf_so3_plan(int N, const double xi[3], int *squarings, int *degree, double *b_scaled);
int qf_launch_so3_taylor(qf_ctx *ctx, const double xi[3], int squarings, int degree, cplx *T);
int qf_launch_so3_grad(qf_ctx *ctx, const cplx *P, cplx *out);

struct qf_oz_job {
    const cplx *X = nullptr;
    const cplx *X_alt = nullptr;
    signed char *planes = nullptr;
    double *scale = nullptr;
};
struct qf_oz_mirror {
    cplx *tbuf = nullptr;
    unsigned *flags = nullptr;
    unsigned epoch = 0;
    int *fault = nullptr;
    const double *diag = nullptr;
    int debug_drop = 0;
};
struct qf_oz_jobs {
    qf_oz_job j[3];
    int n = 0;
    double *diag = nullptr;
};
size_t qf_oz_operand_bytes(int N, int digits);
size_t qf_oz_record_bytes(int N, int digits);
int qf_launch_oz_slice(qf_ctx *ctx, const qf_oz_jobs &jobs, qf_guard guard = qf_guard(), int digits = 0);
int qf_launch_oz_gemm(qf_ctx *ctx, const signed char *pa, const double *sa, const signed char *pm, const double *sm,
                      cplx *C, const qf_epilogue *ep = nullptr, qf_guard guard = qf_guard(), int digits = 0, int digits_m = 0,
                      const double *diag = nullptr);

template <class T> struct qf_same_type { typedef T type; };
template <class T> using qf_same = typename qf_same_type<T>::type;
template <class C>
int qf_launch_update(qf_ctx *ctx, const C *PW, C *W, const C *dW_a, const C *dW_b, C *Whalf, qf_same<C> *kahan_c,
                     int reinitialize, qf_guard guard = qf_guard());
int qf_launch_debug_modulus(qf_ctx *ctx, int n, const double *er, const double *ei, double *out_mod, double *out_sqrt);
int qf_launch_norm_from_rowpart(qf_ctx *ctx, const double *rowpart, int tiles, double *out_dev);
int qf_launch_fold_nonfinite(qf_ctx *ctx, const double *in_dev, double *acc_dev);
int qf_launch_norm_decide(qf_ctx *ctx, const double *rowpart, int tiles, qf_guard guard);
int qf_launch_state_init(qf_ctx *ctx, double tol, int minit, int maxit, const double *norm_dev = nullptr, double tol_factor = 0.0);
template <class C> int qf_launch_norm_inf(qf_ctx *ctx, const C *A, double *out_dev);
int qf_launch_call_begin(qf_ctx *ctx, double tol, int minit, int maxit, int auto_tol, double tol_factor);
template <class C> int qf_launch_inner2(qf_ctx *ctx, const C *A, const C *B, double *out_dev);
int qf_launch_inner(qf_ctx *ctx, const cplx *A, const cplx *B, double *out_dev);
int qf_launch_mhd_sums(qf_ctx *ctx, const cplx *W, const cplx *P, const cplx *Theta, double *part, double *out_dev);
int qf_launch_erk_stage(qf_ctx *ctx, const cplx *A, const cplx *B, double inv_hb, const cplx *W, cplx *acc,
                        double c_acc, cplx *Wp, double c_wp, cplx *Wout, double c_fin);
int qf_launch_magnetic_fix(qf_ctx *ctx, const cplx *BTP, const cplx *BT, cplx *dW, const cplx *dW_old, const cplx *W,
                           cplx *Whalf, double *rowpart);
int qf_launch_magnetic_update(qf_ctx *ctx, const cplx *BT, cplx *W, const cplx *dW, cplx *Whalf);
// ... 7 lines not shown
```

### quflow_amd/csrc/zgemm.hip

```cpp
#include "qf_internal.h"
#include "qf_step_end.h"

#include <cstring>

typedef double v4d __attribute__((ext_vector_type(4)));

#ifdef QF_STAMP
__device__ unsigned long long *qf_stamp_buf = nullptr;
#define QF_STAMP_SLOTS 80
#ifdef QF_STAMP_LIGHT
#define QF_STAMP_AT(slot_)
#define QF_STAMP_PH(kt_, ph_)
__device__ unsigned long long *qf_phase_buf = nullptr;
#else
#define QF_STAMP_AT(slot_)                                                              \
    if (qf_stamp_buf && lane == 0 && (slot_) < QF_STAMP_SLOTS)                          \
        qf_stamp_buf[((size_t)blockIdx.x * (T / 64) + wave) * QF_STAMP_SLOTS + (slot_)] = __builtin_amdgcn_s_memtime();
__device__ unsigned long long *qf_phase_buf = nullptr;
#define QF_STAMP_PH(kt_, ph_)                                                           \
    if (qf_phase_buf && tid == 0 && (kt_) >= 20 && (kt_) < 28)                          \
        qf_phase_buf[((size_t)blockIdx.x * 8 + ((kt_) - 20)) * 5 + (ph_)] = __builtin_amdgcn_s_memtime();
#endif
__device__ unsigned long long *qf_tri_buf = nullptr;
#define QF_TRI_STAMP(seg_, k_)                                                          \
// ... 71 lines not shown
    static constexpr size_t bytes = main_bytes > epi_bytes ? main_bytes : epi_bytes;
};

__device__ __forceinline__ int xcd_remap(int bid, int nwg)
{
    const int q = nwg / 8, r = nwg % 8, xcd = bid % 8;
    return (xcd < r ? xcd * (q + 1) : r * (q + 1) + (xcd - r) * q) + bid / 8;
}

template <int BM, int BN, int WM, int WN, bool EPI, bool EXACT, bool FUSED = false>
__global__ __launch_bounds__(WM *WN * 64) void k_zgemm(int N, int tiles_m, int tiles_n,
                                                        const cplx *__restrict__ A,
                                                        const cplx *__restrict__ B, cplx *__restrict__ C,
                                                        qf_epilogue ep, qf_guard guard)
{
    constexpr int T = WM * WN * 64;
    constexpr bool FAST = EXACT && BM == 64 && BN == 64 && T == 256;
    using SM = tile_smem<BM, BN, FAST>;
    constexpr int WTM = BM / WM, WTN = BN / WN;
    constexpr int MT = WTM / 16, NT = WTN / 16;
    constexpr int A_STRIDE = SM::A_STRIDE, B_STRIDE = SM::B_STRIDE;
    constexpr int A_PER = (BM * BK) / T;
    constexpr int B_PER = (BN * BK) / T;
    constexpr int A_ROWS_PER = T / BK;
    constexpr int B_ROWS_PER = T / BN;
    static_assert((BM * BK) % T == 0 && (BN * BK) % T == 0 && T % BK == 0 && T % BN == 0, "tile/threads mismatch");
    constexpr int A3_STRIDE = SM::A3_STRIDE, B3_STRIDE = SM::B3_STRIDE;

    extern __shared__ __attribute__((aligned(16))) unsigned char smem_raw[];

    const int tid = (int)threadIdx.x;
    const int lane = tid & 63, wave = tid >> 6;
    const int wm = wave / WN, wn = wave % WN;
    const int r16 = lane & 15, q4 = lane >> 4;

    int tm, tn;
    if (QF_XCD_BLOCK && tiles_m % 4 == 0 && tiles_n % 2 == 0) {
        const int x = blockIdx.x & 7, l = blockIdx.x >> 3;
        const int R = tiles_m / 4, C = tiles_n / 2;
        int lr, lc;
        if (R % 4 == 0 && C % 8 == 0) {
            const int blk = l >> 5, in = l & 31;
            const int bpr = C / 8;
            lr = (blk / bpr) * 4 + (in >> 3);
            lc = (blk % bpr) * 8 + (in & 7);
        } else {
            lr = l / C;
            lc = l % C;
        }
        tm = (x >> 1) * R + lr;
        tn = (x & 1) * C + lc;
    } else {
        const int lid0 = xcd_remap(blockIdx.x, tiles_m * tiles_n);
        tm = lid0 / tiles_n;
        tn = lid0 % tiles_n;
    }
    const int lid = tm * tiles_n + tn;
    const int i0 = tm * BM, j0 = tn * BN;
    const cplx zero = make_double2(0.0, 0.0);
    const int parity = (EPI && guard.state) ? guard.state->dw_parity : 0;
    const cplx *__restrict__ ep_dW_old = ep.dW[parity];
    cplx *__restrict__ ep_dW_new = ep.dW[parity ^ 1];
    const int wpar = (FUSED && guard.state) ? guard.state->w_parity : 0;
    const cplx *__restrict__ ep_W = FUSED ? (wpar ? ep.Wpair[1] : ep.Wpair[0]) : ep.W;
    cplx *__restrict__ ep_Wnext = FUSED ? (wpar ? ep.Wpair[0] : ep.Wpair[1]) : nullptr;

    const unsigned char *lds_fa[2] = {
        smem_raw + (size_t)(q4 * A_STRIDE + wm * WTM + (r16 ^ q4)) * sizeof(cplx),
        smem_raw + (size_t)(q4 * A_STRIDE + wm * WTM + (r16 ^ q4 ^ 4)) * sizeof(cplx)};
    const unsigned char *lds_fb = smem_raw + SM::B_OFFSET + (size_t)(q4 * B_STRIDE + wn * WTN + r16) * sizeof(cplx);
    unsigned char *lds_sa = smem_raw + (size_t)((tid % BK) * A_STRIDE + ((tid / BK) ^ (tid % BK & 7))) * sizeof(cplx);
    unsigned char *lds_sb = smem_raw + SM::B_OFFSET + (size_t)tid * sizeof(cplx);
    const unsigned char *lds_fa3[2] = {
        smem_raw + SM::A3_OFFSET + (size_t)(q4 * A3_STRIDE + (FAST ? wm * WTM + 2 * (r16 ^ q4) : wm * WTM + r16)) * sizeof(double),
        smem_raw + SM::A3_OFFSET + (size_t)(q4 * A3_STRIDE + (FAST ? wm * WTM + 2 * (r16 ^ q4 ^ 4) : wm * WTM + r16)) * sizeof(double)};
    const unsigned char *lds_fb3 = smem_raw + SM::B3_OFFSET +
        (size_t)(q4 * B3_STRIDE + (FAST ? wn * WTN + 2 * r16 : wn * WTN + r16)) * sizeof(double);
    unsigned char *lds_sa3 = smem_raw + SM::A3_OFFSET +
        (size_t)((tid % BK) * A3_STRIDE + (FAST ? 2 * ((tid / BK) ^ (tid % BK & 7)) : tid / BK)) * sizeof(double);
    const int b_jA = ((tid % 32) / 16) * 32 + (tid % 16);
    unsigned char *lds_sb3 = smem_raw + SM::B3_OFFSET +
        (size_t)(FAST ? (tid / 32) * B3_STRIDE + 32 * ((tid % 32) / 16) + 2 * (tid % 16) : tid) * sizeof(double);
    if (FAST) lds_sb = smem_raw + SM::B_OFFSET + (size_t)((tid / 32) * B_STRIDE + b_jA) * sizeof(cplx);

    const unsigned a_voff = (unsigned)(((size_t)(tid / BK) * N + (tid % BK)) * sizeof(cplx));
    const unsigned b_voff = (unsigned)(((size_t)(tid / BN) * N + (tid % BN)) * sizeof(cplx));
    const int kt_off = 0;
    const unsigned char *a_row = reinterpret_cast<const unsigned char *>(A) + (size_t)i0 * N * sizeof(cplx);
    const size_t a_pass = (size_t)A_ROWS_PER * N * sizeof(cplx);
    const size_t b_pass = (size_t)B_ROWS_PER * N * sizeof(cplx);
    const size_t b_ktile = (size_t)BK * N * sizeof(cplx);
    const __amdgpu_buffer_rsrc_t rsrcA = __builtin_amdgcn_make_buffer_rsrc(
        const_cast<cplx *>(A), 0, FAST ? (int)((size_t)N * N * sizeof(cplx)) : 0, 0x00020000);
    const unsigned fa_voff = (unsigned)(((size_t)(tid / BK) * N + (tid % BK)) * sizeof(cplx));
    const unsigned fb_voff = (unsigned)(((size_t)(tid / 32) * N + b_jA) * sizeof(cplx));
    const unsigned fa_soff0 = (unsigned)((size_t)i0 * N * sizeof(cplx));
    const unsigned fb_soff0 = (unsigned)((size_t)j0 * sizeof(cplx));
    const unsigned f_rows16 = (unsigned)((size_t)16 * N * sizeof(cplx));
    typedef unsigned v4u __attribute__((ext_vector_type(4)));

    cplx e_c[EPI ? MT : 1][EPI ? NT : 1][4], e_t[EPI ? MT : 1][EPI ? NT : 1][4];
    cplx e_w[EPI ? MT : 1][EPI ? NT : 1][4], e_old[EPI ? MT : 1][EPI ? NT : 1][4];
#define QF_EPI_COMM                                                                    \
    {                                                                                  \
        _Pragma("unroll") for (int mi = 0; mi < MT; ++mi)                              \
            _Pragma("unroll") for (int ni = 0; ni < NT; ++ni)                          \
                _Pragma("unroll") for (int reg = 0; reg < 4; ++reg)                    \
        {                                                                              \
            e_c[mi][ni][reg].x = e_c[mi][ni][reg].x - e_t[mi][ni][reg].x;              \
            e_c[mi][ni][reg].y = e_c[mi][ni][reg].y + e_t[mi][ni][reg].y;              \
        }                                                                              \
    }
#define QF_EPI_FETCH(dst_, src_, TRANSPOSED_)                                          \
    {                                                                                  \
        _Pragma("unroll") for (int mi = 0; mi < MT; ++mi)                              \
            _Pragma("unroll") for (int ni = 0; ni < NT; ++ni)                          \
                _Pragma("unroll") for (int reg = 0; reg < 4; ++reg)                    \
        {                                                                              \
            const int gi = i0 + wm * WTM + mi * 16 + q4 + 4 * reg;                     \
            const int gj = j0 + wn * WTN + ni * 16 + r16;                              \
            dst_[mi][ni][reg] = zero;                                                  \
            if (EXACT || (gi < N && gj < N))                                           \
                dst_[mi][ni][reg] = (TRANSPOSED_) ? (src_)[(size_t)gj * N + gi] : (src_)[(size_t)gi * N + gj]; \
        }                                                                              \
    }

    v4d accR[MT][NT], accI[MT][NT], accS[MT][NT];
#pragma unroll
    for (int a = 0; a < MT; ++a)
#pragma unroll
        for (int b = 0; b < NT; ++b) {
            accR[a][b] = (v4d){0.0, 0.0, 0.0, 0.0};
            accI[a][b] = (v4d){0.0, 0.0, 0.0, 0.0};
            accS[a][b] = (v4d){0.0, 0.0, 0.0, 0.0};
        }

    cplx ra[2][A_PER], rb[2][B_PER];
    cplx fa[2][MT], fb[2][NT];
    double fas[2][MT], fbs[2][NT];

#define QF_TAIL_STEADY_HERE (QF_TAIL_LITERAL && EXACT && (FAST || QF_TAIL_LITERAL32))
#define QF_KT_CLAMP(kt_) ((QF_TAIL_STEADY_HERE && (kt_) >= KT) ? KT - 1 : (kt_))
#define QF_LOAD_TILE_A(kt_, SET_)                                                      \
    if (FAST) {                                                                        \
        const unsigned sa = fa_soff0 + (unsigned)QF_KT_CLAMP(kt_) * (unsigned)(BK * sizeof(cplx)); \
        _Pragma("unroll") for (int r = 0; r < 4; ++r)                                  \
        {                                                                              \
            const v4u t = __builtin_amdgcn_raw_buffer_load_b128(rsrcA, fa_voff, sa + r * f_rows16, 0); \
            ra[SET_][r] = *reinterpret_cast<const cplx *>(&t);                         \
        }                                                                              \
    } else {                                                                           \
        const unsigned char *ap = a_row + (size_t)QF_KT_CLAMP(kt_) * (BK * sizeof(cplx)); \
        _Pragma("unroll") for (int r = 0; r < A_PER; ++r)                              \
        {                                                                              \
            ra[SET_][r] = zero;                                                        \
            if (EXACT || (i0 + tid / BK + r * A_ROWS_PER < N && ((kt_) + kt_off) * BK + tid % BK < N)) \
                ra[SET_][r] = *reinterpret_cast<const cplx *>((ap + r * a_pass) + a_voff); \
        }                                                                              \
    }
#define QF_LOAD_TILE_B(kt_, SET_)                                                      \
    if (FAST) {                                                                        \
        const unsigned sb = fb_soff0 + (unsigned)QF_KT_CLAMP(kt_) * f_rows16;          \
        _Pragma("unroll") for (int r = 0; r < 4; ++r)                                  \
        {                                                                              \
            const v4u t = __builtin_amdgcn_raw_buffer_load_b128(rsrcB, fb_voff + (r & 1) * 256u, sb + (r >> 1) * (f_rows16 / 2), 0); \
            rb[SET_][r] = *reinterpret_cast<const cplx *>(&t);                         \
        }                                                                              \
    } else {                                                                           \
        const unsigned char *bp = b_col + (size_t)QF_KT_CLAMP(kt_) * b_ktile; \
        _Pragma("unroll") for (int r = 0; r < B_PER; ++r)                              \
        {                                                                              \
            rb[SET_][r] = zero;                                                        \
            if (EXACT || (((kt_) + kt_off) * BK + tid / BN + r * B_ROWS_PER < N && j0 + tid % BN < N)) \
                rb[SET_][r] = *reinterpret_cast<const cplx *>((bp + r * b_pass) + b_voff); \
        }                                                                              \
    }
#define QF_LOAD_TILE(kt_, SET_)                                                        \
    {                                                                                  \
        QF_LOAD_TILE_A(kt_, SET_)                                                      \
        QF_LOAD_TILE_B(kt_, SET_)                                                      \
    }
// ... 137 lines not shown
        __builtin_amdgcn_sched_barrier(0);                                             \
         \
        __builtin_amdgcn_s_waitcnt(0xC07F);                                            \
        __builtin_amdgcn_sched_barrier(0);                                             \
        QF_STAMP_AT((kt_) + 2)                                                         \
    }
#define QF_KTILE_PHASE1(kt_, BUF_, STORE_, LOAD_, NEXT_, STEADY_, PREF_)                      \
    {                                                                                  \
                           \
        QF_STAMP_PH(kt_, 0)                                                            \
        QF_READ_FRAGS(1, BUF_, 1)                                                      \
        __builtin_amdgcn_sched_barrier(0);                                             \
        QF_MFMA(0)                                                                     \
        __builtin_amdgcn_sched_barrier(0);                                             \
          \
        QF_STAMP_PH(kt_, 1)                                                            \
        QF_READ_FRAGS(0, BUF_, 2)                                                      \
        __builtin_amdgcn_sched_barrier(0);                                             \
        if ((STORE_) && !QF_ABL_NOSTORE) QF_STORE_TILE((BUF_) ^ 1, (BUF_) ^ 1)         \
        if ((LOAD_) && !QF_ABL_NOGLOAD) QF_LOAD_TILE((kt_) + 3, (BUF_) ^ 1)            \
        if (EPI && (PREF_) == 1) QF_EPI_FETCH(e_c, ep.PW, false)                       \
        if (EPI && (PREF_) == 2) QF_EPI_FETCH(e_t, ep.PW, true)                        \
        if (EPI && (PREF_) == 3) QF_EPI_COMM                                           \
        if (EPI && (PREF_) == 5) {                                                     \
            QF_EPI_FETCH(e_w, ep_W, false)                                             \
            QF_EPI_FETCH(e_old, ep_dW_old, false)                                      \
        }                                                                              \
        QF_MFMA(1)                                                                     \
        if (EXACT && (STEADY_)) {                                                \
              \
            _Pragma("unroll") for (int g = 0; g < (A_PER + B_PER); ++g)                \
            {                                                                          \
                __builtin_amdgcn_sched_group_barrier(SG_MFMA, 1, 0);                   \
                __builtin_amdgcn_sched_group_barrier(SG_DS_WR, 2, 0);                  \
            }                                                                          \
            _Pragma("unroll") for (int g = 0; g < (A_PER + B_PER) / 2; ++g)            \
            {                                                                          \
                __builtin_amdgcn_sched_group_barrier(SG_MFMA, 1, 0);                   \
                __builtin_amdgcn_sched_group_barrier(SG_VMEM_RD, 2, 0);                \
            }                                                                          \
        }                                                                              \
        __builtin_amdgcn_sched_barrier(0);                                             \
                                                                          \
        QF_STAMP_PH(kt_, 2)                                                            \
        QF_READ_FRAGS(1, BUF_, 3)                                                      \
        __builtin_amdgcn_sched_barrier(0);                                             \
        QF_MFMA(0)                                                                     \
        __builtin_amdgcn_sched_barrier(0);                                             \
         \
        if (QF_ABL_NOBARRIER) asm volatile("s_waitcnt lgkmcnt(0)" ::: "memory");      \
        else asm volatile("s_waitcnt lgkmcnt(0)\n\ts_barrier" ::: "memory");           \
        __builtin_amdgcn_sched_barrier(0);                                             \
                                      \
        QF_STAMP_PH(kt_, 3)                                                            \
        if (NEXT_) QF_READ_FRAGS(0, (BUF_) ^ 1, 0)                                     \
        __builtin_amdgcn_sched_barrier(0);                                             \
        QF_MFMA(1)                                                                     \
        __builtin_amdgcn_sched_barrier(0);                                             \
         \
        __builtin_amdgcn_s_waitcnt(0xC07F);                                            \
        __builtin_amdgcn_sched_barrier(0);                                             \
        QF_STAMP_PH(kt_, 4)                                                            \
        QF_STAMP_AT((kt_) + 2)                                                         \
    }
#define QF_KTILE(kt_, BUF_, STORE_, LOAD_, NEXT_, STEADY_, PREF_)                      \
    {                                                                                  \
        if (FAST && QF_STAGE_SPREAD) QF_KTILE_SPREAD(kt_, BUF_, STORE_, LOAD_, NEXT_, STEADY_, PREF_) \
        else QF_KTILE_PHASE1(kt_, BUF_, STORE_, LOAD_, NEXT_, STEADY_, PREF_)          \
    }
#define QF_KTILE_STEADY(kt_, BUF_, PREF_) QF_KTILE(kt_, BUF_, 1, 1, 1, 1, PREF_)
#define QF_KTILE_TAIL(kt_, BUF_) QF_KTILE(kt_, BUF_, ((kt_) + 1 < KT), ((kt_) + 3 < KT), ((kt_) + 1 < KT), 0, 0)
#define QF_KTILE_LAST(kt_, BUF_) QF_KTILE(kt_, BUF_, 0, 0, 0, 0, 5)
#define QF_KLOOP_TAIL(kt_)                                                             \
    {                                                                                  \
        if (QF_TAIL_STEADY_HERE && (kt_) < KT) {     \
            QF_KTILE_STEADY(kt_, 0, 0)                                                 \
            ++(kt_);                                                                   \
        }                                                                              \
        for (; (kt_) < KT; ++(kt_)) {                                                  \
            if ((kt_) & 1) { QF_KTILE_TAIL(kt_, 1) } else { QF_KTILE_TAIL(kt_, 0) }    \
        }                                                                              \
    }

    const int KT = (N + BK - 1) / BK;
    QF_STAMP_AT(0)
    QF_LOAD_TILE_A(0, 0)
    if (KT > 1) { QF_LOAD_TILE_A(1, 1) }
    if (!qf_guard_iter(guard)) return;
    if (!EPI && guard.alt && guard.state->wh_sel) B = static_cast<const cplx *>(guard.alt);
    const unsigned char *b_col = reinterpret_cast<const unsigned char *>(B) + (size_t)j0 * sizeof(cplx);
    const __amdgpu_buffer_rsrc_t rsrcB = __builtin_amdgcn_make_buffer_rsrc(
        const_cast<cplx *>(B), 0, FAST ? (int)((size_t)N * N * sizeof(cplx)) : 0, 0x00020000);
    QF_LOAD_TILE_B(0, 0)
    if (KT > 1) { QF_LOAD_TILE_B(1, 1) }
    QF_STORE_TILE(0, 0)
    __syncthreads();
    if (KT > 2) QF_LOAD_TILE(2, 0)
    QF_READ_FRAGS(0, 0, 0)
    __builtin_amdgcn_s_waitcnt(0xC07F);
    QF_STAMP_AT(1)

    int kt = 0;
    const bool spread = EPI && KT >= 10;
    if (spread) {
        QF_KTILE_STEADY(0, 0, 0)
        QF_KTILE_STEADY(1, 1, 1)
        QF_KTILE_STEADY(2, 0, 2)
        QF_KTILE_STEADY(3, 1, 0)
        QF_KTILE_STEADY(4, 0, 3)
        QF_KTILE_STEADY(5, 1, 0)
        kt = 6;
    }
    for (; kt + ((QF_TAIL_STEADY_HERE) ? 1 : 4) < KT; kt += 2) {
        QF_KTILE_STEADY(kt, 0, 0)
        QF_KTILE_STEADY(kt + 1, 1, 0)
    }
    QF_KLOOP_TAIL(kt)
    if (EPI) {
        if (!spread) {
            QF_EPI_FETCH(e_c, ep.PW, false)
            QF_EPI_FETCH(e_t, ep.PW, true)
            QF_EPI_COMM
        }
        QF_EPI_FETCH(e_w, ep_W, false)
        QF_EPI_FETCH(e_old, ep_dW_old, false)
    }

    if constexpr (!EPI) {
#if QF_WT_PW
        const __amdgpu_buffer_rsrc_t rsrcC = __builtin_amdgcn_make_buffer_rsrc(C, 0, 0x7fffffff, 0x00020000);
#endif
#pragma unroll
        for (int mi = 0; mi < MT; ++mi)
#pragma unroll
            for (int ni = 0; ni < NT; ++ni)
#pragma unroll
                for (int reg = 0; reg < 4; ++reg) {
                    int gi = i0 + wm * WTM + mi * 16 + q4 + 4 * reg;
                    int gj = j0 + wn * WTN + ni * 16 + r16;
                    const double cre = accR[mi][ni][reg] - accI[mi][ni][reg];
                    const double cim = (accS[mi][ni][reg] - accR[mi][ni][reg]) - accI[mi][ni][reg];
                    if (EXACT || (gi < N && gj < N)) {
#if QF_WT_PW
                        const cplx v = make_double2(cre, cim);
                        __builtin_amdgcn_raw_buffer_store_b128(*reinterpret_cast<const v4u *>(&v), rsrcC,
                                                               (unsigned)(((size_t)gi * N + gj) * sizeof(cplx)), 0, 16);
#else
                        C[(size_t)gi * N + gj] = make_double2(cre, cim);
#endif
                    }
                }
    } else {
        double *rs = reinterpret_cast<double *>(smem_raw);
        __syncthreads();
#pragma unroll
        for (int mi = 0; mi < MT; ++mi) {
#pragma unroll
            for (int reg = 0; reg < 4; ++reg) {
                const int li = wm * WTM + mi * 16 + q4 + 4 * reg;
                const int gi = i0 + li;
                double rsum = 0.0;
#pragma unroll
                for (int ni = 0; ni < NT; ++ni) {
                    const int gj = j0 + wn * WTN + ni * 16 + r16;
                    if (EXACT || (gi < N && gj < N)) {
                        const size_t e = (size_t)gi * N + gj;
                        const double cr = e_c[mi][ni][reg].x;
                        const double ci = e_c[mi][ni][reg].y;
                        const double tre = accR[mi][ni][reg] - accI[mi][ni][reg];
                        const double tim = (accS[mi][ni][reg] - accR[mi][ni][reg]) - accI[mi][ni][reg];
                        const double dr = tre + cr;
                        const double di = tim + ci;
                        ep_dW_new[e] = make_double2(dr, di);
                        const cplx w = e_w[mi][ni][reg];
                        ep.Whalf[e] = make_double2(w.x + dr, w.y + di);
                        if (FUSED) {
                            const double wr = w.x + 2.0 * cr, wi = w.y + 2.0 * ci;
                            ep_Wnext[e] = make_double2(wr, wi);
                            ep.Whalf_step[e] = make_double2(wr + dr, wi + di);
                        }
                        const cplx o = e_old[mi][ni][reg];
                        const double er = o.x - dr, ei = o.y - di;
                        rsum += qf_modulus(er, ei);
                    }
                }
                rsum = qf_row16_sum(rsum);
                if (r16 == 0) rs[wn * BM + li] = rsum;
            }
        }
        __syncthreads();
        for (int li = tid; li < BM; li += T) {
            double s = 0.0;
#pragma unroll
            for (int c = 0; c < WN; ++c) s += rs[c * BM + li];
            if (EXACT || i0 + li < N) {
                if (FUSED) __hip_atomic_store(ep.rowpart + (size_t)tn * N + i0 + li, s, __ATOMIC_RELAXED, __HIP_MEMORY_SCOPE_AGENT);
                else ep.rowpart[(size_t)tn * N + i0 + li] = s;
            }
        }
        if (FUSED) {
            asm volatile("s_waitcnt vmcnt(0)" ::: "memory");
            __syncthreads();
            unsigned *last_flag = reinterpret_cast<unsigned *>(rs + WN * BM);
            if (tid == 0) {
                unsigned old = 0u;
                if (!((ep.debug_drop & 2) && lid == 0)) old = __hip_atomic_fetch_add(ep.ticket, 1u, __ATOMIC_RELAXED, __HIP_MEMORY_SCOPE_AGENT);
                *last_flag = (old == (unsigned)(ep.n_tiles - 1)) ? 1u : 0u;
            }
            __syncthreads();
            if (*last_flag != 0u)
                qf_fused_step_end(N, tiles_n, ep.rowpart, ep.ticket, ep.state_rw, ep.rec, guard.iter, tid, rs + WN * BM + 2);
        }
    }
    QF_STAMP_AT(KT + 2)
}

constexpr size_t TRI_SMEM_BYTES = 2 * 64 * 65 * sizeof(cplx) + 4 * 64 * sizeof(double) + 64;

__global__ __launch_bounds__(256) void k_zgemm_tri(int N, int nt, int U, int E, const cplx *__restrict__ A,
                                                    const cplx *__restrict__ B, qf_epilogue ep, qf_guard guard,
                                                    qf_streamk sk)
{
    constexpr int BM = 64, BN = 64, WM = 2, WN = 2;
    constexpr bool EPI = true, EXACT = true, FAST = true;
    using SM = tile_smem<BM, BN, true>;
    constexpr int T = WM * WN * 64;
    constexpr int WTM = BM / WM, WTN = BN / WN;
    constexpr int MT = WTM / 16, NT = WTN / 16;
    constexpr int A_STRIDE = SM::A_STRIDE, B_STRIDE = SM::B_STRIDE;
    constexpr int A_PER = (BM * BK) / T, B_PER = (BN * BK) / T;
    constexpr int A_ROWS_PER = T / BK, B_ROWS_PER = T / BN;
    constexpr int A3_STRIDE = SM::A3_STRIDE, B3_STRIDE = SM::B3_STRIDE;
    constexpr int TS = BN + 1;
    constexpr int TT_BYTES = BM * TS * (int)sizeof(cplx);
    static_assert((size_t)2 * TT_BYTES + (WN * BM + WM * BN) * sizeof(double) + 16 <= TRI_SMEM_BYTES, "epilogue scratch exceeds the LDS request");
    static_assert(TRI_SMEM_BYTES >= SM::main_bytes, "K-loop buffers exceed the LDS request");
    typedef unsigned v4u __attribute__((ext_vector_type(4)));
    constexpr int SG_MFMA = 0x008, SG_VMEM_RD = 0x020, SG_DS_WR = 0x200;

    extern __shared__ __attribute__((aligned(16))) unsigned char smem_raw[];

    const int tid = threadIdx.x;
    const int lane = tid & 63, wave = tid >> 6;
    const int wm = wave / WN, wn = wave % WN;
    const int r16_c = lane & 15, q4_c = lane >> 4;
    const int G = gridDim.x;
    const int c = xcd_remap(blockIdx.x, G);
    const int KTN = N / BK;
    const int S = KTN + E;
    int u = (int)((long long)c * U / G);
    const int u_end = (int)((long long)(c + 1) * U / G);
    const cplx zero = make_double2(0.0, 0.0);

    const unsigned char *lds_fa[2] = {
        smem_raw + (size_t)(q4_c * A_STRIDE + wm * WTM + (r16_c ^ q4_c)) * sizeof(cplx),
        smem_raw + (size_t)(q4_c * A_STRIDE + wm * WTM + (r16_c ^ q4_c ^ 4)) * sizeof(cplx)};
    const unsigned char *lds_fb = smem_raw + SM::B_OFFSET + (size_t)(q4_c * B_STRIDE + wn * WTN + r16_c) * sizeof(cplx);
    unsigned char *lds_sa = smem_raw + (size_t)((tid % BK) * A_STRIDE + ((tid / BK) ^ (tid % BK & 7))) * sizeof(cplx);
    const unsigned char *lds_fa3[2] = {
        smem_raw + SM::A3_OFFSET + (size_t)(q4_c * A3_STRIDE + wm * WTM + 2 * (r16_c ^ q4_c)) * sizeof(double),
        smem_raw + SM::A3_OFFSET + (size_t)(q4_c * A3_STRIDE + wm * WTM + 2 * (r16_c ^ q4_c ^ 4)) * sizeof(double)};
    const unsigned char *lds_fb3 = smem_raw + SM::B3_OFFSET + (size_t)(q4_c * B3_STRIDE + wn * WTN + 2 * r16_c) * sizeof(double);
    unsigned char *lds_sa3 = smem_raw + SM::A3_OFFSET + (size_t)((tid % BK) * A3_STRIDE + 2 * ((tid / BK) ^ (tid % BK & 7))) * sizeof(double);
    const int b_jA = ((tid % 32) / 16) * 32 + (tid % 16);
    unsigned char *lds_sb3 = smem_raw + SM::B3_OFFSET + (size_t)((tid / 32) * B3_STRIDE + 32 * ((tid % 32) / 16) + 2 * (tid % 16)) * sizeof(double);
    unsigned char *lds_sb = smem_raw + SM::B_OFFSET + (size_t)((tid / 32) * B_STRIDE + b_jA) * sizeof(cplx);
    const __amdgpu_buffer_rsrc_t rsrcA = __builtin_amdgcn_make_buffer_rsrc(const_cast<cplx *>(A), 0, (int)((size_t)N * N * sizeof(cplx)), 0x00020000);
    const __amdgpu_buffer_rsrc_t rsrcB = __builtin_amdgcn_make_buffer_rsrc(const_cast<cplx *>(B), 0, (int)((size_t)N * N * sizeof(cplx)), 0x00020000);
    const unsigned fa_voff = (unsigned)(((size_t)(tid / BK) * N + (tid % BK)) * sizeof(cplx));
    const unsigned fb_voff = (unsigned)(((size_t)(tid / 32) * N + b_jA) * sizeof(cplx));
    const unsigned f_rows16 = (unsigned)((size_t)16 * N * sizeof(cplx));
    const __amdgpu_buffer_rsrc_t rsrcP = __builtin_amdgcn_make_buffer_rsrc(sk.partial, 0, (int)((size_t)sk.slots * (BM * BN) * sizeof(cplx)), 0x00020000);
    const unsigned p_voff = (unsigned)(tid * sizeof(cplx));
    const unsigned char *a_row = nullptr, *b_col = nullptr;
    const size_t a_pass = 0, b_pass = 0, b_ktile = 0;
    const unsigned a_voff = 0, b_voff = 0;
    const int kt_off = 0;
    const int i0 = 0, j0 = 0;

    cplx e_c[MT][NT][4], e_t[MT][NT][4], e_w[MT][NT][4], e_old[MT][NT][4];
    v4d accR[MT][NT], accI[MT][NT], accS[MT][NT];
    cplx ra[2][A_PER], rb[2][B_PER];
    cplx fa[2][MT], fb[2][NT];
    double fas[2][MT], fbs[2][NT];
#pragma unroll
    for (int r = 0; r < A_PER; ++r) ra[1][r] = rb[1][r] = zero;

#define QF_TRI_KOF(p_) ((p_) <= 0 ? 0 : ((p_) <= E + 1 ? 1 : ((p_) - E > KTN ? KTN : (int)((p_) - E))))
#define QF_TRI_NEXT(u_, found_, t_, k0_, KT_, tm_, tn_)                                \
    {                                                                                  \
        found_ = false;                                                                \
        while (!(found_) && (u_) < u_end) {                                            \
            t_ = (int)((u_) / S);                                                      \
            const int pa_ = (u_) - (t_) * S;                                           \
            int pb_ = u_end - (t_) * S;                                                \
            if (pb_ > S) pb_ = S;                                                      \
            const int klo_ = QF_TRI_KOF(pa_), khi_ = QF_TRI_KOF(pb_);                  \
            u_ = (t_) * S + pb_;                                                       \
            if (klo_ < khi_) {                                                         \
                found_ = true;                                                         \
                k0_ = klo_;                                                            \
                KT_ = khi_ - klo_;                                                     \
                int rem_ = (t_);                                                       \
                tm_ = 0;                                                               \
                while (rem_ >= nt - (tm_)) { rem_ -= nt - (tm_); ++(tm_); }            \
                tn_ = (tm_) + rem_;                                                    \
            }                                                                          \
        }                                                                              \
    }
#define QF_TRI_START_LOADS(k0_, KT_, tm_, tn_)                                         \
    {                                                                                  \
        const int kt_of_segment_ = (KT_);                                              \
        fa_soff0 = (unsigned)(((size_t)(tm_) * BM * N + (size_t)(k0_) * BK) * sizeof(cplx)); \
        fb_soff0 = (unsigned)(((size_t)(k0_) * BK * N + (size_t)(tn_) * BN) * sizeof(cplx)); \
        {                                                                              \
            const int KT = kt_of_segment_;        \
            QF_LOAD_TILE(0, 0)                                                         \
            if (KT > 1) { QF_LOAD_TILE(1, 1) }                                         \
        }                                                                              \
    }
    int seg = 0;
    (void)seg;
    bool run_finale = false;
    int t = 0, k0 = 0, KT = 0, tm = 0, tn = 0;
    unsigned fa_soff0 = 0, fb_soff0 = 0;
    bool have = false;
    QF_TRI_NEXT(u, have, t, k0, KT, tm, tn)
    if (have) QF_TRI_START_LOADS(k0, KT, tm, tn)
    if (!qf_guard_iter(guard)) have = false;
    const int parity = guard.state ? guard.state->dw_parity : 0;
    const cplx *__restrict__ ep_dW_old = ep.dW[parity];
    cplx *__restrict__ ep_dW_new = ep.dW[parity ^ 1];
    const int wpar = (ep.fused && guard.state) ? guard.state->w_parity : 0;
    const cplx *__restrict__ ep_W = ep.fused ? ep.Wpair[wpar] : ep.W;
    cplx *__restrict__ ep_Wnext = ep.fused ? ep.Wpair[wpar ^ 1] : nullptr;
    const bool below_maxit = ep.fused && sk.state_rw && (guard.iter + 1 < sk.state_rw->maxit);
    const bool open_for_sure = below_maxit && (guard.iter + 1 < sk.state_rw->minit);
    const bool open_if_large = below_maxit && guard.iter == 0;
    const double tol_now = (ep.fused && sk.state_rw) ? sk.state_rw->tol : 0.0;

    while (have) {
        const int i0 = tm * BM, j0 = tn * BN;
        const bool head = (k0 == 0);
        int r16 = r16_c, q4 = q4_c, lane_v = lane;
        asm volatile("" : "+v"(r16), "+v"(q4), "+v"(lane_v));
#pragma unroll
        for (int a = 0; a < MT; ++a)
#pragma unroll
            for (int b = 0; b < NT; ++b) {
                accR[a][b] = (v4d){0.0, 0.0, 0.0, 0.0};
                accI[a][b] = (v4d){0.0, 0.0, 0.0, 0.0};
                accS[a][b] = (v4d){0.0, 0.0, 0.0, 0.0};
            }

        QF_TRI_STAMP(seg, 0)
        QF_TRI_NOTE(seg, 4, k0)
        QF_TRI_NOTE(seg, 5, KT)
        QF_STORE_TILE(0, 0)
        __syncthreads();
        if (KT > 2) { QF_LOAD_TILE(2, 0) }
        QF_READ_FRAGS(0, 0, 0)
        __builtin_amdgcn_s_waitcnt(0xC07F);

        QF_TRI_STAMP(seg, 6)
        int kt = 0;
        const bool spread = head && KT >= 10;
        if (spread) {
            QF_KTILE_STEADY(0, 0, 0)
            QF_KTILE_STEADY(1, 1, 1)
            QF_KTILE_STEADY(2, 0, 2)
            QF_KTILE_STEADY(3, 1, 0)
            QF_KTILE_STEADY(4, 0, 3)
            QF_KTILE_STEADY(5, 1, 0)
            kt = 6;
        }
        for (; kt + (QF_TAIL_STEADY_HERE ? 1 : 4) < KT; kt += 2) {
            QF_KTILE_STEADY(kt, 0, 0)
            QF_KTILE_STEADY(kt + 1, 1, 0)
        }
        QF_KLOOP_TAIL(kt)
        QF_TRI_STAMP(seg, 1)

        int n_t = 0, n_k0 = 0, n_KT = 0, n_tm = 0, n_tn = 0;
        bool have_next = false;
        QF_TRI_NEXT(u, have_next, n_t, n_k0, n_KT, n_tm, n_tn)

        if (!head) {
            const int park_slot = c;
#pragma unroll
            for (int mi = 0; mi < MT; ++mi)
#pragma unroll
                for (int ni = 0; ni < NT; ++ni)
#pragma unroll
                    for (int reg = 0; reg < 4; ++reg) {
                        const cplx v = make_double2(accR[mi][ni][reg] - accI[mi][ni][reg],
                                                    (accS[mi][ni][reg] - accR[mi][ni][reg]) - accI[mi][ni][reg]);
                        __builtin_amdgcn_raw_buffer_store_b128(*reinterpret_cast<const v4u *>(&v), rsrcP,
                                                               p_voff + (unsigned)(((mi * NT + ni) * 4 + reg) * T * sizeof(cplx)),
                                                               (unsigned)((size_t)park_slot * (BM * BN) * sizeof(cplx)), QF_SK_AUX_ST);
                    }
            asm volatile("s_waitcnt vmcnt(0)" ::: "memory");
            if (have_next) QF_TRI_START_LOADS(n_k0, n_KT, n_tm, n_tn)
            __syncthreads();
            if (tid == 0 && !(sk.debug_drop & 1)) __hip_atomic_store(sk.flags + park_slot, sk.epoch, __ATOMIC_RELAXED, __HIP_MEMORY_SCOPE_AGENT);
            QF_TRI_STAMP(seg, 2)
        } else {
            if (!spread) {
                QF_EPI_FETCH(e_c, ep.PW, false)
                QF_EPI_FETCH(e_t, ep.PW, true)
                QF_EPI_COMM
            }
            QF_EPI_FETCH(e_w, ep_W, false)
            QF_EPI_FETCH(e_old, ep_dW_old, false)
            double tre[MT][NT][4], tim[MT][NT][4];
#pragma unroll
            for (int mi = 0; mi < MT; ++mi)
#pragma unroll
                for (int ni = 0; ni < NT; ++ni)
#pragma unroll
                    for (int reg = 0; reg < 4; ++reg) {
                        tre[mi][ni][reg] = accR[mi][ni][reg] - accI[mi][ni][reg];
                        tim[mi][ni][reg] = (accS[mi][ni][reg] - accR[mi][ni][reg]) - accI[mi][ni][reg];
                    }
            if (KT < KTN) {
                const int tile_org = t * S, tile_end = tile_org + S;
                const int c_first = c + 1;
                int c_last = c;
                while (c_last + 1 < G && (int)((long long)(c_last + 1) * U / G) < tile_end) ++c_last;
#define QF_TRI_HAS_PIECE(c2_)                                                          \
    (QF_TRI_KOF((int)((long long)(c2_) * U / G) - tile_org) <                          \
     QF_TRI_KOF(((int)(((long long)(c2_) + 1) * U / G) < tile_end ? (int)(((long long)(c2_) + 1) * U / G) : tile_end) - tile_org))
                for (int c2 = c_last; c2 >= c_first; --c2) {
                    const int slot2 = c2;
                    if (!QF_TRI_HAS_PIECE(c2)) continue;
                    if (tid == 0) {
                        unsigned spins = 0;
                        while (__hip_atomic_load(sk.flags + slot2, __ATOMIC_RELAXED, __HIP_MEMORY_SCOPE_AGENT) != sk.epoch) {
                            __builtin_amdgcn_s_sleep(QF_POLL_SLEEP);
                            if (++spins > sk.spin_limit) {
                                *sk.fault = 1;
                                break;
                            }
                        }
                    }
                    asm volatile("s_barrier" ::: "memory");
                    const unsigned soff = (unsigned)((size_t)slot2 * (BM * BN) * sizeof(cplx));
                    cplx v[MT * NT * 4];
#pragma unroll
                    for (int q = 0; q < MT * NT * 4; ++q) {
                        const v4u raw = __builtin_amdgcn_raw_buffer_load_b128(rsrcP, p_voff + (unsigned)(q * T * sizeof(cplx)), soff, QF_SK_AUX_LD);
                        v[q] = *reinterpret_cast<const cplx *>(&raw);
                    }
#pragma unroll
                    for (int mi = 0; mi < MT; ++mi)
#pragma unroll
                        for (int ni = 0; ni < NT; ++ni)
#pragma unroll
                            for (int reg = 0; reg < 4; ++reg) {
                                tre[mi][ni][reg] += v[(mi * NT + ni) * 4 + reg].x;
                                tim[mi][ni][reg] += v[(mi * NT + ni) * 4 + reg].y;
                            }
                }
            }
            QF_TRI_STAMP(seg, 2)
            cplx *Th = reinterpret_cast<cplx *>(smem_raw);
            cplx *Ts = reinterpret_cast<cplx *>(smem_raw + TT_BYTES);
            double *rs = reinterpret_cast<double *>(smem_raw + 2 * TT_BYTES);
            double *cs = rs + WN * BM;
            unsigned *open_flag = reinterpret_cast<unsigned *>(cs + WM * BN);
            const bool offdiag = (tm != tn);
            asm volatile("s_waitcnt lgkmcnt(0)\n\ts_barrier" ::: "memory");

            double csum[NT] = {0.0, 0.0};
            if (tid == 0) *open_flag = 0u;
#pragma unroll
            for (int mi = 0; mi < MT; ++mi) {
#pragma unroll
                for (int reg = 0; reg < 4; ++reg) {
                    const int li = wm * WTM + mi * 16 + q4 + 4 * reg;
                    double rsum = 0.0;
#pragma unroll
                    for (int ni = 0; ni < NT; ++ni) {
                        const int lj = wn * WTN + ni * 16 + r16;
                        const size_t e = (size_t)(i0 + li) * N + (j0 + lj);
                        const double dr = tre[mi][ni][reg] + e_c[mi][ni][reg].x;
                        const double di = tim[mi][ni][reg] + e_c[mi][ni][reg].y;
                        tre[mi][ni][reg] = dr;
                        tim[mi][ni][reg] = di;
                        const cplx w = e_w[mi][ni][reg];
                        const cplx wh = make_double2(w.x + dr, w.y + di);
                        ep_dW_new[e] = make_double2(dr, di);
                        ep.Whalf[e] = wh;
                        Th[li * TS + lj] = wh;
                        if (!ep.fused) Ts[li * TS + lj] = make_double2(dr, di);
                        const cplx o = e_old[mi][ni][reg];
                        const double er = o.x - dr, ei = o.y - di;
                        const double a = qf_modulus(er, ei);
                        rsum += a;
                        csum[ni] += a;
                    }
                    rsum = qf_row16_sum(rsum);
                    if (r16 == 0) rs[wn * BM + li] = rsum;
                }
            }
            if (offdiag) {
#pragma unroll
                for (int ni = 0; ni < NT; ++ni) {
                    double s2 = csum[ni];
                    s2 += __shfl_xor(s2, 16, 64);
                    s2 += __shfl_xor(s2, 32, 64);
                    if (q4 == 0) cs[wm * BN + wn * WTN + ni * 16 + r16] = s2;
                }
            }
            asm volatile("s_waitcnt lgkmcnt(0)\n\ts_barrier" ::: "memory");
            if (tid < BM) {
                double s2 = 0.0;
#pragma unroll
                for (int cc = 0; cc < WN; ++cc) s2 += rs[cc * BM + tid];
                __hip_atomic_store(ep.rowpart + (size_t)tn * N + i0 + tid, s2, __ATOMIC_RELAXED, __HIP_MEMORY_SCOPE_AGENT);
                if (open_if_large && s2 > tol_now) *open_flag = 1u;
            } else if (offdiag && tid < BM + BN) {
                const int lj = tid - BM;
                double s2 = 0.0;
#pragma unroll
                for (int cc = 0; cc < WM; ++cc) s2 += cs[cc * BN + lj];
                __hip_atomic_store(ep.rowpart + (size_t)tm * N + j0 + lj, s2, __ATOMIC_RELAXED, __HIP_MEMORY_SCOPE_AGENT);
                if (open_if_large && s2 > tol_now) *open_flag = 1u;
            }
            unsigned ticket_old = 0u;
            if (ep.fused) {
                asm volatile("s_waitcnt vmcnt(0) lgkmcnt(0)\n\ts_barrier" ::: "memory");
                if (tid == 0 && !((sk.debug_drop & 2) && t == 0))
                    ticket_old = __hip_atomic_fetch_add(sk.ticket, 1u, __ATOMIC_RELAXED, __HIP_MEMORY_SCOPE_AGENT);
            } else {
                asm volatile("s_waitcnt lgkmcnt(0)\n\ts_barrier" ::: "memory");
            }
            QF_TRI_STAMP(seg, 7)
            const bool speculate = ep.fused && !(open_for_sure || (open_if_large && *open_flag != 0u));

            if (speculate) {
#pragma unroll
                for (int mi = 0; mi < MT; ++mi)
#pragma unroll
                    for (int reg = 0; reg < 4; ++reg) {
                        const int li = wm * WTM + mi * 16 + q4 + 4 * reg;
#pragma unroll
                        for (int ni = 0; ni < NT; ++ni) {
                            const int lj = wn * WTN + ni * 16 + r16;
                            const size_t e = (size_t)(i0 + li) * N + (j0 + lj);
                            const cplx w = e_w[mi][ni][reg];
                            const cplx wc = make_double2(w.x + 2.0 * e_c[mi][ni][reg].x, w.y + 2.0 * e_c[mi][ni][reg].y);
                            const cplx whs = make_double2(wc.x + tre[mi][ni][reg], wc.y + tim[mi][ni][reg]);
                            ep_Wnext[e] = wc;
                            ep.Whalf_step[e] = whs;
                            Ts[li * TS + lj] = whs;
                        }
                    }
            }
            asm volatile("s_waitcnt lgkmcnt(0)\n\ts_barrier" ::: "memory");
            if (offdiag) {
#pragma unroll
                for (int r = 0; r < 16; ++r) {
                    const int jl = wave * 16 + r;
                    const cplx wv = Th[lane_v * TS + jl];
                    const size_t e2 = (size_t)(j0 + jl) * N + (i0 + lane_v);
                    ep.Whalf[e2] = make_double2(-wv.x, wv.y);
                    if (speculate || !ep.fused) {
                        const cplx ws = Ts[lane_v * TS + jl];
                        if (ep.fused) ep.Whalf_step[e2] = make_double2(-ws.x, ws.y);
                        else ep_dW_new[e2] = make_double2(-ws.x, ws.y);
                    }
                }
            }
            if (have_next) QF_TRI_START_LOADS(n_k0, n_KT, n_tm, n_tn)
            if (ep.fused) {
                unsigned *last_flag = reinterpret_cast<unsigned *>(rs);
                if (tid == 0) *last_flag = (ticket_old == (unsigned)(sk.n_tiles - 1)) ? 1u : 0u;
                asm volatile("s_waitcnt lgkmcnt(0)\n\ts_barrier" ::: "memory");
                if (*last_flag != 0u) run_finale = true;
            }
        }
        QF_TRI_STAMP(seg, 3)
        ++seg;
        have = have_next;
        t = n_t;
        k0 = n_k0;
        KT = n_KT;
        tm = n_tm;
        tn = n_tn;
        asm volatile("s_waitcnt lgkmcnt(0)\n\ts_barrier" ::: "memory");
    }
    if (run_finale)
        qf_fused_step_end(N, nt, ep.rowpart, sk.ticket, sk.state_rw, sk.rec, guard.iter, tid, reinterpret_cast<double *>(smem_raw));
#undef QF_TRI_NEXT
#undef QF_TRI_KOF
#undef QF_TRI_HAS_PIECE
#undef QF_TRI_START_LOADS
}

template <bool EXACT>
__global__ __launch_bounds__(256) void k_zgemm_tri32(int N, int nt, const cplx *__restrict__ A, const cplx *__restrict__ B,
                                                      qf_epilogue ep, qf_guard guard, qf_tri32 sx)
{
    if (!qf_guard_iter(guard)) return;
    constexpr int BM = 32, BN = 32, WM = 2, WN = 2;
    constexpr bool EPI = true, FAST = false;
    using SM = tile_smem<BM, BN, false>;
    constexpr int T = WM * WN * 64;
    constexpr int WTM = BM / WM, WTN = BN / WN;
    constexpr int MT = WTM / 16, NT = WTN / 16;
    static_assert(MT == 1 && NT == 1, "one MFMA tile per wave");
    constexpr int A_STRIDE = SM::A_STRIDE, B_STRIDE = SM::B_STRIDE;
    constexpr int A_PER = (BM * BK) / T, B_PER = (BN * BK) / T;
    constexpr int A_ROWS_PER = T / BK, B_ROWS_PER = T / BN;
    constexpr int A3_STRIDE = SM::A3_STRIDE, B3_STRIDE = SM::B3_STRIDE;
    constexpr int TS = BN + 1;
    constexpr int TT_BYTES = BM * TS * (int)sizeof(cplx);
    static_assert((size_t)2 * TT_BYTES + (WN * BM + WM * BN) * sizeof(double) + 16 <= SM::bytes, "epilogue scratch exceeds the K-loop buffers");
    typedef unsigned v4u __attribute__((ext_vector_type(4)));
    constexpr int SG_MFMA = 0x008, SG_VMEM_RD = 0x020, SG_DS_WR = 0x200;

    extern __shared__ __attribute__((aligned(16))) unsigned char smem_raw[];

    const int tid = threadIdx.x;
    const int lane = tid & 63, wave = tid >> 6;
    const int wm = wave / WN, wn = wave % WN;
    const int r16 = lane & 15, q4 = lane >> 4;

    const int n_diag_w = nt * sx.split_diag;
    const int n_off = nt * (nt - 1) / 2;
    int tm, tn, h, nh, t;
    if ((int)blockIdx.x < n_diag_w) {
        nh = sx.split_diag;
        tm = tn = (int)blockIdx.x % nt;
        h = (int)blockIdx.x / nt;
        t = tm;
    } else {
        const int nw = (int)gridDim.x - n_diag_w;
        const int w = (n_diag_w % 8 == 0) ? xcd_remap((int)blockIdx.x - n_diag_w, nw) : (int)blockIdx.x - n_diag_w;
        nh = sx.split;
        const int o = w % n_off;
        h = w / n_off;
        tm = 0;
        int rem = o;
        while (rem >= nt - 1 - tm) {
            rem -= nt - 1 - tm;
            ++tm;
        }
        tn = tm + 1 + rem;
        t = nt + o;
    }
    const int i0 = tm * BM, j0 = tn * BN;
    const int KTN = (N + BK - 1) / BK;
    const int kt_begin = (int)((long long)h * KTN / nh);
    const int KT = (int)((long long)(h + 1) * KTN / nh) - kt_begin;

    const cplx zero = make_double2(0.0, 0.0);
    const int parity = guard.state ? guard.state->dw_parity : 0;
    const cplx *__restrict__ ep_dW_old = ep.dW[parity];
    cplx *__restrict__ ep_dW_new = ep.dW[parity ^ 1];
    const int wpar = (ep.fused && guard.state) ? guard.state->w_parity : 0;
    const cplx *__restrict__ ep_W = ep.fused ? ep.Wpair[wpar] : ep.W;
    cplx *__restrict__ ep_Wnext = ep.fused ? ep.Wpair[wpar ^ 1] : nullptr;
    const bool below_maxit = ep.fused && sx.state_rw && (guard.iter + 1 < sx.state_rw->maxit);
    const bool open_for_sure = below_maxit && (guard.iter + 1 < sx.state_rw->minit);
    const bool open_if_large = below_maxit && guard.iter == 0;
    const double tol_now = (ep.fused && sx.state_rw) ? sx.state_rw->tol : 0.0;

    const unsigned char *lds_fa[2] = {
        smem_raw + (size_t)(q4 * A_STRIDE + wm * WTM + (r16 ^ q4)) * sizeof(cplx),
        smem_raw + (size_t)(q4 * A_STRIDE + wm * WTM + (r16 ^ q4 ^ 4)) * sizeof(cplx)};
    const unsigned char *lds_fb = smem_raw + SM::B_OFFSET + (size_t)(q4 * B_STRIDE + wn * WTN + r16) * sizeof(cplx);
    unsigned char *lds_sa = smem_raw + (size_t)((tid % BK) * A_STRIDE + ((tid / BK) ^ (tid % BK & 7))) * sizeof(cplx);
    unsigned char *lds_sb = smem_raw + SM::B_OFFSET + (size_t)tid * sizeof(cplx);
    const unsigned char *lds_fa3[2] = {
        smem_raw + SM::A3_OFFSET + (size_t)(q4 * A3_STRIDE + wm * WTM + r16) * sizeof(double),
        smem_raw + SM::A3_OFFSET + (size_t)(q4 * A3_STRIDE + wm * WTM + r16) * sizeof(double)};
    const unsigned char *lds_fb3 = smem_raw + SM::B3_OFFSET + (size_t)(q4 * B3_STRIDE + wn * WTN + r16) * sizeof(double);
    unsigned char *lds_sa3 = smem_raw + SM::A3_OFFSET + (size_t)((tid % BK) * A3_STRIDE + tid / BK) * sizeof(double);
    unsigned char *lds_sb3 = smem_raw + SM::B3_OFFSET + (size_t)tid * sizeof(double);
// ... 127 lines not shown
    if (tid < BM) {
        double s2 = 0.0;
#pragma unroll
        for (int cc = 0; cc < WN; ++cc) s2 += rs[cc * BM + tid];
        if (EXACT || i0 + tid < N)
            __hip_atomic_store(ep.rowpart + (size_t)tn * N + i0 + tid, s2, __ATOMIC_RELAXED, __HIP_MEMORY_SCOPE_AGENT);
        if (open_if_large && s2 > tol_now) *open_flag = 1u;
    } else if (offdiag && tid >= 64 && tid < 64 + BN) {
        const int lj = tid - 64;
        double s2 = 0.0;
#pragma unroll
        for (int cc = 0; cc < WM; ++cc) s2 += cs[cc * BN + lj];
        if (EXACT || j0 + lj < N)
            __hip_atomic_store(ep.rowpart + (size_t)tm * N + j0 + lj, s2, __ATOMIC_RELAXED, __HIP_MEMORY_SCOPE_AGENT);
        if (open_if_large && s2 > tol_now) *open_flag = 1u;
    }
    unsigned ticket_old = 0u;
    if (ep.fused && sx.deferred) {
        if (tid == 0 && t == 0 && !(sx.debug_drop & 2)) {
            sx.state_rw->pending_iter = guard.iter;
            sx.state_rw->pending = 1;
        }
        asm volatile("s_waitcnt lgkmcnt(0)\n\ts_barrier" ::: "memory");
    } else if (ep.fused) {
        asm volatile("s_waitcnt vmcnt(0) lgkmcnt(0)\n\ts_barrier" ::: "memory");
        if (tid == 0 && !((sx.debug_drop & 2) && t == 0))
            ticket_old = __hip_atomic_fetch_add(sx.ticket, 1u, __ATOMIC_RELAXED, __HIP_MEMORY_SCOPE_AGENT);
    } else {
        asm volatile("s_waitcnt lgkmcnt(0)\n\ts_barrier" ::: "memory");
    }
    const bool speculate = ep.fused && !(open_for_sure || (open_if_large && *open_flag != 0u));
#pragma unroll
    for (int reg = 0; reg < 4; ++reg) {
        const int li = wm * WTM + q4 + 4 * reg;
        const int lj = wn * WTN + r16;
        const size_t e = (size_t)(i0 + li) * N + (j0 + lj);
        const cplx d = make_double2(tre[reg], tim[reg]);
        const cplx w = e_w[0][0][reg];
        const cplx wh = make_double2(w.x + d.x, w.y + d.y);
        const bool in = EXACT || (i0 + li < N && j0 + lj < N);
        if (in) {
            ep_dW_new[e] = d;
            ep.Whalf[e] = wh;
        }
        Th[li * TS + lj] = wh;
        if (speculate) {
            const cplx wc = make_double2(w.x + 2.0 * e_c[0][0][reg].x, w.y + 2.0 * e_c[0][0][reg].y);
            const cplx whs = make_double2(wc.x + d.x, wc.y + d.y);
            if (in) {
                ep_Wnext[e] = wc;
                ep.Whalf_step[e] = whs;
            }
            Ts[li * TS + lj] = whs;
        } else if (!ep.fused) {
            Ts[li * TS + lj] = d;
        }
    }
    asm volatile("s_waitcnt lgkmcnt(0)\n\ts_barrier" ::: "memory");
    if (offdiag) {
        const int il = lane & 31;
#pragma unroll
        for (int r = 0; r < 4; ++r) {
            const int jl = wave * 8 + r * 2 + (lane >> 5);
            if (!EXACT && (j0 + jl >= N || i0 + il >= N)) continue;
            const cplx wv = Th[il * TS + jl];
            const size_t e2 = (size_t)(j0 + jl) * N + (i0 + il);
            ep.Whalf[e2] = make_double2(-wv.x, wv.y);
            if (speculate || !ep.fused) {
                const cplx ws = Ts[il * TS + jl];
                if (ep.fused) ep.Whalf_step[e2] = make_double2(-ws.x, ws.y);
                else ep_dW_new[e2] = make_double2(-ws.x, ws.y);
            }
        }
    }
    if (ep.fused && !sx.deferred) {
        unsigned *last_flag = reinterpret_cast<unsigned *>(rs);
        if (tid == 0) *last_flag = (ticket_old == (unsigned)(sx.n_tiles - 1)) ? 1u : 0u;
        asm volatile("s_waitcnt lgkmcnt(0)\n\ts_barrier" ::: "memory");
        if (*last_flag != 0u)
            qf_fused_step_end(N, nt, ep.rowpart, sx.ticket, sx.state_rw, sx.rec, guard.iter, tid, reinterpret_cast<double *>(smem_raw));
    }
}

#undef QF_KTILE_STEADY
#undef QF_KTILE_TAIL
#undef QF_KTILE_LAST
#undef QF_KTILE
#undef QF_KTILE_SPREAD
#undef QF_KTILE_PHASE1
#undef QF_STORE_A
#undef QF_STORE_B
#undef QF_EPI_FETCH
#undef QF_EPI_COMM
#undef QF_LOAD_TILE
#undef QF_STORE_TILE
#undef QF_READ_FRAGS
#undef QF_MFMA

struct gemm_cfg {
    int BM, BN;
};

gemm_cfg pick_gemm(int N)
{
    gemm_cfg c;
    bool big;
    if (N % 32 != 0) {
        big = false;
    } else if (N % 64 != 0 || N < 896) {
        big = false;
    } else {
        const long long tiles = (long long)(N / 64) * (N / 64), rounds = (tiles + 255) / 256;
        big = tiles * 100 >= rounds * 256 * 85;
    }
    if (big) { c.BM = 64; c.BN = 64; }
    else { c.BM = 32; c.BN = 32; }
    return c;
}

template <int BM, int BN, int WM, int WN, bool EPI, bool EXACT, bool FUSED>
int launch4(qf_ctx *ctx, const cplx *A, const cplx *B, cplx *C, qf_epilogue ep, const qf_guard &guard)
{
    const int N = ctx->N;
    const int tiles_m = (N + BM - 1) / BM, tiles_n = (N + BN - 1) / BN;
    const size_t smem = tile_smem<BM, BN, EXACT && BM == 64 && BN == 64 && WM * WN == 4>::bytes;
    static qf_smem_attr attr;
    QF_TRY(qf_smem_attr_set(attr, (const void *)k_zgemm<BM, BN, WM, WN, EPI, EXACT, FUSED>, ctx->device, smem));
    if (FUSED) {
        ep.ticket = ctx->ticket + 400;
        ep.n_tiles = tiles_m * tiles_n;
        ep.state_rw = ctx->state;
        ep.rec = ctx->host_rec;
        if (ctx->debug_drop == 2) {
            ep.debug_drop = 2;
            ctx->debug_drop = 0;
        }
    }
    dim3 grid(tiles_m * tiles_n), block(WM * WN * 64);
    qf_plan_note(ctx, 0x1000000ull | (unsigned long long)(BM << 8 | EPI << 2 | EXACT << 1 | (FUSED ? 1 : 0)),
                 "{\"kernel\": \"k_zgemm<%d,%d%s>\", \"arithmetic\": \"fp64 3M, v_mfma_f64_16x16x4_f64\", \"tile\": [%d, %d], "
                 "\"tiles\": %d, \"tile_share\": 1.0, \"workgroups\": %d, \"threads\": %d, \"exact_tiling\": %s, \"step_end\": \"%s\"}",
                 BM, BN, EPI ? ",EPI" : "", BM, BN, tiles_m * tiles_n, tiles_m * tiles_n, WM * WN * 64, EXACT ? "true" : "false",
                 !EPI ? "none" : FUSED ? "fused (last tile decides)" : "two-kernel");
    hipLaunchKernelGGL((k_zgemm<BM, BN, WM, WN, EPI, EXACT, FUSED>), grid, block, smem, ctx->stream, N, tiles_m,
                       tiles_n, A, B, C, ep, guard);
    QF_HIP(hipGetLastError());
    return QF_OK;
}

template <int BM, int BN, int WM, int WN, bool EPI, bool EXACT>
int launch2(qf_ctx *ctx, const cplx *A, const cplx *B, cplx *C, const qf_epilogue &ep, const qf_guard &guard)
{
    if (EPI && ep.fused) return launch4<BM, BN, WM, WN, EPI, EXACT, EPI>(ctx, A, B, C, ep, guard);
    return launch4<BM, BN, WM, WN, EPI, EXACT, false>(ctx, A, B, C, ep, guard);
}

template <int BM, int BN, int WM, int WN>
int launch(qf_ctx *ctx, const cplx *A, const cplx *B, cplx *C, const qf_epilogue *ep, const qf_guard &guard)
{
    const int N = ctx->N;
    const bool exact = (N % BM == 0) && (N % BN == 0) && (N % BK == 0);
    qf_epilogue none;
    if (ep) {
        if (exact) return launch2<BM, BN, WM, WN, true, true>(ctx, A, B, C, *ep, guard);
        return launch2<BM, BN, WM, WN, true, false>(ctx, A, B, C, *ep, guard);
    }
    if (exact) return launch2<BM, BN, WM, WN, false, true>(ctx, A, B, C, none, guard);
    return launch2<BM, BN, WM, WN, false, false>(ctx, A, B, C, none, guard);
}

}

int qf_gemm_tiles_n(int N)
{
    gemm_cfg c = pick_gemm(N);
    return (N + c.BN - 1) / c.BN;
}

int qf_launch_zgemm_tri(qf_ctx *ctx, const cplx *A, const cplx *B, const qf_epilogue *ep, qf_guard guard)
{
    const int N = ctx->N;
    if (!ep || N % 64 != 0 || !ctx->sk_partial || ctx->num_cus < 1) {
        qf_set_error("qf_launch_zgemm_tri: not available for this context (N=%d)", N);
        return QF_ERR_STATE;
    }
    static qf_smem_attr attr;
    QF_TRY(qf_smem_attr_set(attr, (const void *)k_zgemm_tri, ctx->device, TRI_SMEM_BYTES));
    const int nt = N / 64;
    int E = ep->fused ? ctx->sk_epi_units_fused : ctx->sk_epi_units;
    if (E < -8) E = -8;
    const long long units = (long long)nt * (nt + 1) / 2 * (N / BK + E);
    if (units > 0x7fffffffLL) {
        qf_set_error("qf_launch_zgemm_tri: N=%d is too large for the stream-K partition", N);
        return QF_ERR_INVALID;
    }
    long long grid_ll = units / (ctx->sk_min_units > 0 ? ctx->sk_min_units : 1);
    if (grid_ll > ctx->num_cus) grid_ll = ctx->num_cus;
    if (grid_ll < 1) grid_ll = 1;
    const int grid = (int)grid_ll;
    qf_streamk sk;
    const int slots = ctx->sk_slots > 0 ? ctx->sk_slots : ctx->num_cus;
    sk.slots = slots;
    sk.partial = ctx->sk_partial;
    sk.flags = ctx->sk_flags;
    sk.epoch = ++ctx->sk_epoch;
    sk.fault = &ctx->host_rec->fault;
    sk.ticket = ctx->sk_flags + slots;
    sk.n_tiles = nt * (nt + 1) / 2;
    sk.state_rw = ctx->state;
    sk.rec = ctx->host_rec;
    if (ctx->debug_drop == 1 || (ctx->debug_drop == 2 && ep->fused)) {
        sk.debug_drop = ctx->debug_drop;
        sk.spin_limit = 1u << 14;
        ctx->debug_drop = 0;
    }
    qf_plan_note(ctx, 0x2000000ull | (unsigned long long)(grid << 8 | (E & 0x3f) << 1 | (ep->fused ? 1 : 0)),
                 "{\"kernel\": \"k_zgemm_tri\", \"arithmetic\": \"fp64 3M, v_mfma_f64_16x16x4_f64\", \"tile\": [64, 64], \"tiles\": %d, "
                 "\"tile_share\": %.6f, \"workgroups\": %d, \"threads\": 256, \"partition\": \"stream-K over (tile, K-tile) units, "
                 "contiguous ranges, epilogue weight E = %d K-tiles\", \"step_end\": \"%s\"}",
                 sk.n_tiles, (double)sk.n_tiles / ((double)nt * nt), grid, E, ep->fused ? "fused (last finisher decides)" : "two-kernel");
    hipLaunchKernelGGL(k_zgemm_tri, dim3(grid), dim3(256), TRI_SMEM_BYTES, ctx->stream, N, nt, (int)units, E, A, B, *ep, guard, sk);
    QF_HIP(hipGetLastError());
    return QF_OK;
}

int qf_launch_zgemm_tri32(qf_ctx *ctx, const cplx *A, const cplx *B, const qf_epilogue *ep, qf_guard guard)
{
    const int N = ctx->N;
    if (!ep || N < 64 || !ctx->t32_partial || !ctx->t32_arrive) {
        qf_set_error("qf_launch_zgemm_tri32: not available for this context (N=%d)", N);
        return QF_ERR_STATE;
    }
    const int nt = (N + 31) / 32;
    qf_tri32 sx;
    sx.partial = ctx->t32_partial;
    sx.arrive = ctx->t32_arrive;
    sx.split = (ctx->tri32_split == 2 || ctx->tri32_split == 4) ? ctx->tri32_split : 1;
    sx.split_diag = (ctx->tri32_split_diag == 2 || ctx->tri32_split_diag == 4) ? ctx->tri32_split_diag : 1;
    while (sx.split > 1 && (N + BK - 1) / BK / sx.split < 2) sx.split >>= 1;
    while (sx.split_diag > 1 && (N + BK - 1) / BK / sx.split_diag < 2) sx.split_diag >>= 1;
    sx.ticket = ctx->ticket + 401;
    sx.n_tiles = nt * (nt + 1) / 2;
    sx.state_rw = ctx->state;
    sx.rec = ctx->host_rec;
    if (ctx->debug_drop == 2 && ep->fused) {
        sx.debug_drop = 2;
        ctx->debug_drop = 0;
    }
    sx.deferred = (ep->fused && ctx->defer && guard.state) ? 1 : 0;
    const int grid = nt * sx.split_diag + nt * (nt - 1) / 2 * sx.split;
    const size_t smem = tile_smem<32, 32, false>::bytes;
    qf_plan_note(ctx, 0x3000000ull | (unsigned long long)(grid << 6 | sx.split << 3 | sx.split_diag << 1 | sx.deferred),
                 "{\"kernel\": \"k_zgemm_tri32<%s>\", \"arithmetic\": \"fp64 3M, v_mfma_f64_16x16x4_f64\", \"tile\": [32, 32], \"tiles\": %d, "
                 "\"tile_share\": %.6f, \"workgroups\": %d, \"threads\": 256, \"partition\": \"K range of an off-diagonal / diagonal tile in "
                 "%d / %d pieces, one workgroup each\", \"step_end\": \"%s\"}",
                 N % 32 == 0 ? "exact" : "guarded edges", sx.n_tiles, (double)sx.n_tiles / ((double)nt * nt), grid, sx.split, sx.split_diag,
                 !ep->fused ? "two-kernel" : sx.deferred ? "deferred (the next solve's workgroups decide)" : "fused (last tile decides)");
    if (N % 32 == 0) hipLaunchKernelGGL(k_zgemm_tri32<true>, dim3(grid), dim3(256), smem, ctx->stream, N, nt, A, B, *ep, guard, sx);
    else hipLaunchKernelGGL(k_zgemm_tri32<false>, dim3(grid), dim3(256), smem, ctx->stream, N, nt, A, B, *ep, guard, sx);
    QF_HIP(hipGetLastError());
    return QF_OK;
}

int qf_launch_zgemm(qf_ctx *ctx, const cplx *A, const cplx *B, cplx *C, const qf_epilogue *ep, qf_guard guard)
{
    if (ep && ctx->gemm_tri) return qf_launch_zgemm_tri(ctx, A, B, ep, guard);
    if (ep && ctx->gemm_tri32) return qf_launch_zgemm_tri32(ctx, A, B, ep, guard);
    gemm_cfg c = pick_gemm(ctx->N);
    if (c.BM == 64) return launch<64, 64, 2, 2>(ctx, A, B, C, ep, guard);
    return launch<32, 32, 2, 2>(ctx, A, B, C, ep, guard);
}
```

Before: 2687.

## Keep Whalf as upper tiles only and read transposed tiles in first product

The stream-K triangular product stops mirroring Whalf into its lower triangle. The first product Phalf*Whalf instead loads the B operand by its upper tiles, reading transposed tiles and negating them through skew-Hermitian symmetry when a lower tile is needed. This removes the mirror writes, the extra LDS barrier in the fused epilogue and some global traffic per iteration. In exchange the GEMM kernel gains a transposed-B load and store path, and Whalf must be mirrored once at exit. It is enabled by default when the tri path is active and N is a multiple of 64.

```diff
diff --git a/include/quflow_hip.h b/include/quflow_hip.h
--- a/include/quflow_hip.h
+++ b/include/quflow_hip.h
@@ -189,6 +189,7 @@
 int qf_debug_modulus(qf_ctx *ctx, int n, const double *er_host, const double *ei_host, double *out_modulus_host,
                      double *out_sqrt_host);
 int qf_zgemm(qf_ctx *ctx, const void *A_host, const void *B_host, void *C_host);
+int qf_zgemm_upper(qf_ctx *ctx, const void *A_host, const void *B_host, void *C_host);
 int qf_commutator(qf_ctx *ctx, const void *W_host, const void *P_host, void *C_host, int skewherm);
 int qf_zgemm_i8(qf_ctx *ctx, const void *A_host, const void *B_host, void *C_host);
 int qf_fixedpoint_products(qf_ctx *ctx, const void *Phalf_host, const void *Whalf_host, const void *W_host,
diff --git a/quflow_amd/_lib.py b/quflow_amd/_lib.py
--- a/quflow_amd/_lib.py
+++ b/quflow_amd/_lib.py
@@ -169,6 +169,7 @@
     "qf_download_buffer": (ctypes.c_int, [_vp, ctypes.c_int, _vp]),
     "qf_debug_guard_check": (ctypes.c_int, [ctypes.POINTER(ctypes.c_longlong), ctypes.POINTER(ctypes.c_longlong), ctypes.c_char_p, ctypes.c_int]),
     "qf_zgemm": (ctypes.c_int, [_vp, _vp, _vp, _vp]),
+    "qf_zgemm_upper": (ctypes.c_int, [_vp, _vp, _vp, _vp]),
     "qf_commutator": (ctypes.c_int, [_vp, _vp, _vp, _vp, ctypes.c_int]),
     "qf_zgemm_i8": (ctypes.c_int, [_vp, _vp, _vp, _vp]),
     "qf_fixedpoint_products": (ctypes.c_int, [_vp, _vp, _vp, _vp, _vp, ctypes.c_int, _vp, _vp, _vp]),
diff --git a/quflow_amd/csrc/api_context.hip b/quflow_amd/csrc/api_context.hip
--- a/quflow_amd/csrc/api_context.hip
+++ b/quflow_amd/csrc/api_context.hip
@@ -139,6 +139,7 @@
     if (const char *g = getenv("QUFLOW_HIP_I8_MIN_N")) ctx->gemm_i8_min_n = atoi(g);
     if (const char *g = getenv("QUFLOW_HIP_TRI_MIN_N")) ctx->gemm_tri_min_n = atoi(g);
     if (const char *g = getenv("QUFLOW_HIP_DEFER")) ctx->defer_allowed = !(g[0] == '0');
+    if (const char *g = getenv("QUFLOW_HIP_WHALF_MIRROR")) ctx->whalf_mirror = (g[0] == '1');
     if (getenv("QUFLOW_HIP_DEBUG"))
         if (const char *g = getenv("QUFLOW_HIP_DEBUG_DROP_FLAG")) ctx->debug_drop = atoi(g);
     if (const char *g = getenv("QUFLOW_HIP_FACTOR_CACHE_MB")) ctx->factor_budget_bytes = (size_t)(atoi(g) > 0 ? atoi(g) : 1) << 20;
diff --git a/quflow_amd/csrc/api_isomp.hip b/quflow_amd/csrc/api_isomp.hip
--- a/quflow_amd/csrc/api_isomp.hip
+++ b/quflow_amd/csrc/api_isomp.hip
@@ -205,11 +205,14 @@
         }
         {
             prof_scope p(ctx, QF_KERNEL_GEMM1);
+            if constexpr (!is_c64<S>) g.b_upper = ctx->whalf_upper ? 1 : 0;
             QF_TRY(launch_gemm(ctx, w->Phalf, w->Whalf, w->PW, nullptr, g));
+            g.b_upper = 0;
         }
         {
             prof_scope p(ctx, QF_KERNEL_GEMM2);
-            const auto ep = epilogue_of(w, true);
+            auto ep = epilogue_of(w, true);
+            if constexpr (!is_c64<S>) ep.whalf_upper_only = ctx->whalf_upper ? 1 : 0;
             g.alt = nullptr;
             if constexpr (is_c64<S>) {
                 if (w->tri) QF_TRY(qf_launch_cgemm_tri(ctx, w->PW, w->Phalf, &ep, g));
@@ -502,6 +505,7 @@
     } else {
         QF_TRY(select_second_product(ctx));
         ctx->defer = ctx->defer_allowed && !ctx->gemm_i8 && ctx->gemm_tri32 && ctx->N <= 512;
+        ctx->whalf_upper = !ctx->whalf_mirror && ctx->gemm_tri && !ctx->gemm_i8 && qf_gemm_b_upper_ok(ctx->N);
     }
     w->increment_is_zero = !carry;
     w->increment_valid = true;
@@ -537,6 +541,11 @@
         QF_TRY(qf_launch_mirror_lower(ctx, w->W));
         QF_TRY(qf_launch_mirror_lower(ctx, w->dW[w->dw_cur]));
     }
+    if constexpr (!is_c64<S>)
+        if (ctx->whalf_upper && steps > 0) {
+            QF_TRY(qf_launch_mirror_lower(ctx, w->Whalf));
+            ctx->whalf_upper = false;
+        }
     if constexpr (!is_c64<S>)
         if (ctx->diag_at_exit) {
             QF_TRY(qf_enqueue_diagnostics(ctx));
@@ -925,7 +934,12 @@
         return QF_ERR_INVALID;
     }
     const int variant_arg = variant;
+    const bool upper = (variant & 16) != 0;
     variant &= 15;
+    if (upper && variant != 1) {
+        qf_set_error("qf_fixedpoint_products: variant bit 4 (Whalf by its upper tiles) goes with the stream-K product (kind 1)");
+        return QF_ERR_INVALID;
+    }
     if (variant == 1 && !ctx->sk_partial) {
         qf_set_error("qf_fixedpoint_products: the upper-triangle product needs N %% 64 == 0 (N=%d)", ctx->N);
         return QF_ERR_INVALID;
@@ -943,9 +957,11 @@
     QF_HIP(hipMemcpyAsync(ctx->Whalf, Whalf_host, bytes, hipMemcpyHostToDevice, ctx->stream));
     QF_HIP(hipMemcpyAsync(ctx->stage, W_host, bytes, hipMemcpyHostToDevice, ctx->stream));
     QF_HIP(hipMemcpyAsync(ctx->dW[0], dW_old_host, bytes, hipMemcpyHostToDevice, ctx->stream));
-    QF_TRY(qf_launch_zgemm(ctx, ctx->Phalf, ctx->Whalf, ctx->PW, nullptr));
+    if (upper) QF_TRY(qf_launch_zgemm_b_upper(ctx, ctx->Phalf, ctx->Whalf, ctx->PW));
+    else QF_TRY(qf_launch_zgemm(ctx, ctx->Phalf, ctx->Whalf, ctx->PW, nullptr));
     qf_epilogue ep = epilogue_of(ctx, false);
     ep.W = ctx->stage;
+    ep.whalf_upper_only = upper ? 1 : 0;
     const bool saved = ctx->gemm_tri, saved32 = ctx->gemm_tri32;
     const int s_min = ctx->sk_min_units, s_epi = ctx->sk_epi_units, s_so = ctx->tri32_split, s_sd = ctx->tri32_split_diag;
     ctx->gemm_tri = (variant == 1);
diff --git a/quflow_amd/csrc/api_transforms.hip b/quflow_amd/csrc/api_transforms.hip
--- a/quflow_amd/csrc/api_transforms.hip
+++ b/quflow_amd/csrc/api_transforms.hip
@@ -415,6 +415,22 @@
     return QF_OK;
 }
 
+int qf_zgemm_upper(qf_ctx *ctx, const void *A_host, const void *B_host, void *C_host)
+{
+    QF_TRY(check_ctx(ctx));
+    if (!A_host || !B_host || !C_host) {
+        qf_set_error("qf_zgemm_upper: null buffer");
+        return QF_ERR_INVALID;
+    }
+    const size_t bytes = (size_t)ctx->N * ctx->N * sizeof(cplx);
+    QF_HIP(hipMemcpyAsync(ctx->stage, A_host, bytes, hipMemcpyHostToDevice, ctx->stream));
+    QF_HIP(hipMemcpyAsync(ctx->Phalf, B_host, bytes, hipMemcpyHostToDevice, ctx->stream));
+    QF_TRY(qf_launch_zgemm_b_upper(ctx, ctx->stage, ctx->Phalf, ctx->PW));
+    QF_HIP(hipMemcpyAsync(C_host, ctx->PW, bytes, hipMemcpyDeviceToHost, ctx->stream));
+    QF_HIP(hipStreamSynchronize(ctx->stream));
+    return QF_OK;
+}
+
 int qf_commutator(qf_ctx *ctx, const void *W_host, const void *P_host, void *C_host, int skewherm)
 {
     QF_TRY(check_ctx(ctx));
diff --git a/quflow_amd/csrc/qf_internal.h b/quflow_amd/csrc/qf_internal.h
--- a/quflow_amd/csrc/qf_internal.h
+++ b/quflow_amd/csrc/qf_internal.h
@@ -93,6 +93,7 @@
     int step = 0;
     int iter = 0;
     const void *alt = nullptr;
+    int b_upper = 0;
 };
 
 #ifdef __HIPCC__
@@ -374,6 +375,8 @@
     bool gemm_tri_allowed = true;
     bool gemm_tri = false;
     int gemm_tri_min_n = 960;
+    bool whalf_mirror = false;
+    bool whalf_upper = false;
     bool gemm_tri32 = false;
     int tri32_split = 2, tri32_split_diag = 1;
     cplx *t32_partial = nullptr;
@@ -399,7 +402,7 @@
     int profile_stride = 1;
     struct plan_slot {
         unsigned long long key = 0;
-        char text[384] = {0};
+        char text[512] = {0};
     } plan[QF_KERNEL_COUNT];
     int plan_role = -1;
     long long prof_seen[QF_KERNEL_COUNT] = {0};
@@ -472,6 +475,7 @@
     qf_dev_state *state_rw = nullptr;
     qf_host_record *rec = nullptr;
     int debug_drop = 0;
+    int whalf_upper_only = 0;
 };
 struct qf_streamk {
     cplx *partial = nullptr;
@@ -499,6 +503,8 @@
     int deferred = 0;
 };
 int qf_gemm_tiles_n(int N);
+bool qf_gemm_b_upper_ok(int N);
+int qf_launch_zgemm_b_upper(qf_ctx *ctx, const cplx *A, const cplx *B, cplx *C, qf_guard guard = qf_guard());
 int qf_launch_zgemm_tri32(qf_ctx *ctx, const cplx *A, const cplx *B, const qf_epilogue *ep, qf_guard guard = qf_guard());
 int qf_launch_zgemm_tri(qf_ctx *ctx, const cplx *A, const cplx *B, const qf_epilogue *ep, qf_guard guard = qf_guard());
 int qf_launch_zgemm(qf_ctx *ctx, const cplx *A, const cplx *B, cplx *C, const qf_epilogue *ep,
diff --git a/quflow_amd/csrc/zgemm.hip b/quflow_amd/csrc/zgemm.hip
--- a/quflow_amd/csrc/zgemm.hip
+++ b/quflow_amd/csrc/zgemm.hip
@@ -177,6 +177,14 @@
     unsigned char *lds_sb3 = smem_raw + SM::B3_OFFSET +
         (size_t)(FAST ? (tid / 32) * B3_STRIDE + 32 * ((tid % 32) / 16) + 2 * (tid % 16) : tid) * sizeof(double);
     if (FAST) lds_sb = smem_raw + SM::B_OFFSET + (size_t)((tid / 32) * B_STRIDE + b_jA) * sizeof(cplx);
+    const unsigned char *lds_fbT[2] = {
+        smem_raw + SM::B_OFFSET + (size_t)(q4 * B_STRIDE + wn * WTN + (r16 ^ q4)) * sizeof(cplx),
+        smem_raw + SM::B_OFFSET + (size_t)(q4 * B_STRIDE + wn * WTN + (r16 ^ q4 ^ 4)) * sizeof(cplx)};
+    const unsigned char *lds_fb3T[2] = {
+        smem_raw + SM::B3_OFFSET + (size_t)(q4 * B3_STRIDE + wn * WTN + 2 * (r16 ^ q4)) * sizeof(double),
+        smem_raw + SM::B3_OFFSET + (size_t)(q4 * B3_STRIDE + wn * WTN + 2 * (r16 ^ q4 ^ 4)) * sizeof(double)};
+    unsigned char *lds_sbT = smem_raw + SM::B_OFFSET + (size_t)((tid % BK) * B_STRIDE + ((tid / BK) ^ (tid % BK & 7))) * sizeof(cplx);
+    unsigned char *lds_sb3T = smem_raw + SM::B3_OFFSET + (size_t)((tid % BK) * B3_STRIDE + 2 * ((tid / BK) ^ (tid % BK & 7))) * sizeof(double);
 
     const unsigned a_voff = (unsigned)(((size_t)(tid / BK) * N + (tid % BK)) * sizeof(cplx));
     const unsigned b_voff = (unsigned)(((size_t)(tid / BN) * N + (tid % BN)) * sizeof(cplx));
@@ -192,6 +200,7 @@
     const unsigned fa_soff0 = (unsigned)((size_t)i0 * N * sizeof(cplx));
     const unsigned fb_soff0 = (unsigned)((size_t)j0 * sizeof(cplx));
     const unsigned f_rows16 = (unsigned)((size_t)16 * N * sizeof(cplx));
+    const unsigned fbt_soff0 = (unsigned)((size_t)j0 * N * sizeof(cplx));
     typedef unsigned v4u __attribute__((ext_vector_type(4)));
 
     cplx e_c[EPI ? MT : 1][EPI ? NT : 1][4], e_t[EPI ? MT : 1][EPI ? NT : 1][4];
@@ -495,6 +504,98 @@
         }                                                                              \
     }
 
+#define QF_LOAD_TILE_BX(kt_, SET_, BT_)                                                \
+    if (BT_) {                                                                         \
+        const unsigned sb = fbt_soff0 + (unsigned)QF_KT_CLAMP(kt_) * (unsigned)(BK * sizeof(cplx)); \
+        _Pragma("unroll") for (int r = 0; r < 4; ++r)                                  \
+        {                                                                              \
+            const v4u t = __builtin_amdgcn_raw_buffer_load_b128(rsrcB, fa_voff, sb + r * f_rows16, 0); \
+            rb[SET_][r] = *reinterpret_cast<const cplx *>(&t);                         \
+        }                                                                              \
+    } else {                                                                           \
+        QF_LOAD_TILE_B(kt_, SET_)                                                      \
+    }
+#define QF_STORE_BX(BUF_, SET_, BT_)                                                   \
+    if (BT_) {                                                                         \
+        _Pragma("unroll") for (int r = 0; r < 4; ++r)                                  \
+            *reinterpret_cast<cplx *>(lds_sbT + (BUF_) * SM::B_BUF_BYTES + r * 16 * (int)sizeof(cplx)) = rb[SET_][r]; \
+        _Pragma("unroll") for (int h = 0; h < 2; ++h)                                  \
+            *reinterpret_cast<double2 *>(lds_sb3T + (BUF_) * SM::B3_BUF_BYTES + h * 32 * (int)sizeof(double)) =            \
+                make_double2(rb[SET_][2 * h].y - rb[SET_][2 * h].x, rb[SET_][2 * h + 1].y - rb[SET_][2 * h + 1].x); \
+    } else {                                                                           \
+        QF_STORE_B(BUF_, SET_)                                                         \
+    }
+#define QF_READ_FRAGS_X(SET_, BUF_, K4_, BT_)                                          \
+    if (BT_) {                                                                         \
+        _Pragma("unroll") for (int mi = 0; mi < MT; ++mi)                              \
+            fa[SET_][mi] = *reinterpret_cast<const cplx *>(                            \
+                lds_fa[(K4_) & 1] + (BUF_) * SM::A_BUF_BYTES + ((K4_) * 4 * A_STRIDE + mi * 16) * (int)sizeof(cplx)); \
+        _Pragma("unroll") for (int ni = 0; ni < NT; ++ni)                              \
+            fb[SET_][ni] = *reinterpret_cast<const cplx *>(                            \
+                lds_fbT[(K4_) & 1] + (BUF_) * SM::B_BUF_BYTES + ((K4_) * 4 * B_STRIDE + ni * 16) * (int)sizeof(cplx)); \
+        const double2 sa2 = *reinterpret_cast<const double2 *>(                        \
+            lds_fa3[(K4_) & 1] + (BUF_) * SM::A3_BUF_BYTES + (K4_) * 4 * A3_STRIDE * (int)sizeof(double)); \
+        const double2 sb2 = *reinterpret_cast<const double2 *>(                        \
+            lds_fb3T[(K4_) & 1] + (BUF_) * SM::B3_BUF_BYTES + (K4_) * 4 * B3_STRIDE * (int)sizeof(double)); \
+        fas[SET_][0] = sa2.x;                                                          \
+        fas[SET_][MT - 1] = sa2.y;                                                     \
+        fbs[SET_][0] = sb2.x;                                                          \
+        fbs[SET_][NT - 1] = sb2.y;                                                     \
+    } else {                                                                           \
+        QF_READ_FRAGS(SET_, BUF_, K4_)                                                 \
+    }
+#define QF_KTILE_X(kt_, BUF_, CUR_, NXT_, LD_)                                         \
+    {                                                                                  \
+                                               \
+        QF_READ_FRAGS_X(1, BUF_, 1, CUR_)                                              \
+        __builtin_amdgcn_sched_barrier(0);                                             \
+        QF_STORE_A((BUF_) ^ 1, (BUF_) ^ 1)                                             \
+        QF_MFMA(0)                                                                     \
+        _Pragma("unroll") for (int g = 0; g < (A_PER * 3) / 2; ++g)                    \
+        {                                                                              \
+            __builtin_amdgcn_sched_group_barrier(SG_MFMA, 2, 0);                       \
+            __builtin_amdgcn_sched_group_barrier(SG_DS_WR, 1, 0);                      \
+        }                                                                              \
+        __builtin_amdgcn_sched_barrier(0);                                             \
+                                                              \
+        QF_READ_FRAGS_X(0, BUF_, 2, CUR_)                                              \
+        __builtin_amdgcn_sched_barrier(0);                                             \
+        QF_STORE_BX((BUF_) ^ 1, (BUF_) ^ 1, NXT_)                                      \
+        QF_MFMA(1)                                                                     \
+        _Pragma("unroll") for (int g = 0; g < (B_PER * 3) / 2; ++g)                    \
+        {                                                                              \
+            __builtin_amdgcn_sched_group_barrier(SG_MFMA, 2, 0);                       \
+            __builtin_amdgcn_sched_group_barrier(SG_DS_WR, 1, 0);                      \
+        }                                                                              \
+        __builtin_amdgcn_sched_barrier(0);                                             \
+                              \
+        QF_READ_FRAGS_X(1, BUF_, 3, CUR_)                                              \
+        __builtin_amdgcn_sched_barrier(0);                                             \
+        QF_LOAD_TILE_A((kt_) + 3, (BUF_) ^ 1)                                          \
+        QF_LOAD_TILE_BX((kt_) + 3, (BUF_) ^ 1, LD_)                                    \
+        QF_MFMA(0)                                                                     \
+        _Pragma("unroll") for (int g = 0; g < A_PER + B_PER; ++g)                      \
+        {                                                                              \
+            __builtin_amdgcn_sched_group_barrier(SG_MFMA, 1, 0);                       \
+            __builtin_amdgcn_sched_group_barrier(SG_VMEM_RD, 1, 0);                    \
+        }                                                                              \
+        __builtin_amdgcn_sched_barrier(0);                                             \
+        asm volatile("s_waitcnt lgkmcnt(0)\n\ts_barrier" ::: "memory");                \
+        __builtin_amdgcn_sched_barrier(0);                                             \
+                                      \
+        QF_READ_FRAGS_X(0, (BUF_) ^ 1, 0, NXT_)                                        \
+        __builtin_amdgcn_sched_barrier(0);                                             \
+        QF_MFMA(1)                                                                     \
+        __builtin_amdgcn_sched_barrier(0);                                             \
+        __builtin_amdgcn_s_waitcnt(0xC07F);                                            \
+        __builtin_amdgcn_sched_barrier(0);                                             \
+    }
+#define QF_NEGATE_T1                                                                   \
+    {                                                                                  \
+        _Pragma("unroll") for (int mi = 0; mi < MT; ++mi)                              \
+            _Pragma("unroll") for (int ni = 0; ni < NT; ++ni) accR[mi][ni] = -accR[mi][ni]; \
+    }
+
     const int KT = (N + BK - 1) / BK;
     QF_STAMP_AT(0)
     QF_LOAD_TILE_A(0, 0)
@@ -514,6 +615,25 @@
     QF_STAMP_AT(1)
 
     int kt = 0;
+    if constexpr (FAST && !EPI && QF_STAGE_SPREAD == 1 && QF_TAIL_LITERAL) {
+        if (guard.b_upper && tn + 1 < tiles_n) {
+            const int KB = (tn + 1) * (BN / BK);
+            for (; kt + 4 < KB; kt += 2) {
+                QF_KTILE_X(kt, 0, 0, 0, 0)
+                QF_KTILE_X(kt + 1, 1, 0, 0, 0)
+            }
+            QF_KTILE_X(kt, 0, 0, 0, 0)
+            QF_KTILE_X(kt + 1, 1, 0, 0, 1)
+            QF_KTILE_X(kt + 2, 0, 0, 0, 1)
+            QF_KTILE_X(kt + 3, 1, 0, 1, 1)
+            QF_NEGATE_T1
+            for (kt = KB; kt + 1 < KT; kt += 2) {
+                QF_KTILE_X(kt, 0, 1, 1, 1)
+                QF_KTILE_X(kt + 1, 1, 1, 1, 1)
+            }
+            QF_NEGATE_T1
+        }
+    }
     const bool spread = EPI && KT >= 10;
     if (spread) {
         QF_KTILE_STEADY(0, 0, 0)
@@ -630,9 +750,10 @@
 
 constexpr size_t TRI_SMEM_BYTES = 2 * 64 * 65 * sizeof(cplx) + 4 * 64 * sizeof(double) + 64;
 
-__global__ __launch_bounds__(256) void k_zgemm_tri(int N, int nt, int U, int E, const cplx *__restrict__ A,
-                                                    const cplx *__restrict__ B, qf_epilogue ep, qf_guard guard,
-                                                    qf_streamk sk)
+template <bool WH_UP>
+__device__ __forceinline__ void zgemm_tri_body(int N, int nt, int U, int E, const cplx *__restrict__ A,
+                                               const cplx *__restrict__ B, const qf_epilogue &ep, const qf_guard &guard,
+                                               const qf_streamk &sk)
 {
     constexpr int BM = 64, BN = 64, WM = 2, WN = 2;
     constexpr bool EPI = true, EXACT = true, FAST = true;
@@ -751,6 +872,7 @@
     const bool open_for_sure = below_maxit && (guard.iter + 1 < sk.state_rw->minit);
     const bool open_if_large = below_maxit && guard.iter == 0;
     const double tol_now = (ep.fused && sk.state_rw) ? sk.state_rw->tol : 0.0;
+    constexpr bool wh_up = WH_UP;
 
     while (have) {
         const int i0 = tm * BM, j0 = tn * BN;
@@ -904,7 +1026,7 @@
                         const cplx wh = make_double2(w.x + dr, w.y + di);
                         ep_dW_new[e] = make_double2(dr, di);
                         ep.Whalf[e] = wh;
-                        Th[li * TS + lj] = wh;
+                        if (!wh_up) Th[li * TS + lj] = wh;
                         if (!ep.fused) Ts[li * TS + lj] = make_double2(dr, di);
                         const cplx o = e_old[mi][ni][reg];
                         const double er = o.x - dr, ei = o.y - di;
@@ -966,18 +1088,21 @@
                             const cplx whs = make_double2(wc.x + tre[mi][ni][reg], wc.y + tim[mi][ni][reg]);
                             ep_Wnext[e] = wc;
                             ep.Whalf_step[e] = whs;
-                            Ts[li * TS + lj] = whs;
+                            if (!wh_up) Ts[li * TS + lj] = whs;
                         }
                     }
             }
-            asm volatile("s_waitcnt lgkmcnt(0)\n\ts_barrier" ::: "memory");
-            if (offdiag) {
+            const bool mirror_pass = offdiag && !(wh_up && ep.fused);
+            if (!(wh_up && ep.fused)) asm volatile("s_waitcnt lgkmcnt(0)\n\ts_barrier" ::: "memory");
+            if (mirror_pass) {
 #pragma unroll
                 for (int r = 0; r < 16; ++r) {
                     const int jl = wave * 16 + r;
-                    const cplx wv = Th[lane_v * TS + jl];
                     const size_t e2 = (size_t)(j0 + jl) * N + (i0 + lane_v);
-                    ep.Whalf[e2] = make_double2(-wv.x, wv.y);
+                    if (!wh_up) {
+                        const cplx wv = Th[lane_v * TS + jl];
+                        ep.Whalf[e2] = make_double2(-wv.x, wv.y);
+                    }
                     if (speculate || !ep.fused) {
                         const cplx ws = Ts[lane_v * TS + jl];
                         if (ep.fused) ep.Whalf_step[e2] = make_double2(-ws.x, ws.y);
@@ -1009,6 +1134,20 @@
 #undef QF_TRI_KOF
 #undef QF_TRI_HAS_PIECE
 #undef QF_TRI_START_LOADS
+}
+
+__global__ __launch_bounds__(256) void k_zgemm_tri(int N, int nt, int U, int E, const cplx *__restrict__ A,
+                                                    const cplx *__restrict__ B, qf_epilogue ep, qf_guard guard,
+                                                    qf_streamk sk)
+{
+    zgemm_tri_body<false>(N, nt, U, E, A, B, ep, guard, sk);
+}
+
+__global__ __launch_bounds__(256) void k_zgemm_tri_up(int N, int nt, int U, int E, const cplx *__restrict__ A,
+                                                       const cplx *__restrict__ B, qf_epilogue ep, qf_guard guard,
+                                                       qf_streamk sk)
+{
+    zgemm_tri_body<true>(N, nt, U, E, A, B, ep, guard, sk);
 }
 
 template <bool EXACT>
@@ -1302,6 +1441,11 @@
     }
 }
 
+#undef QF_KTILE_X
+#undef QF_NEGATE_T1
+#undef QF_LOAD_TILE_BX
+#undef QF_STORE_BX
+#undef QF_READ_FRAGS_X
 #undef QF_KTILE_STEADY
 #undef QF_KTILE_TAIL
 #undef QF_KTILE_LAST
@@ -1357,11 +1501,17 @@
         }
     }
     dim3 grid(tiles_m * tiles_n), block(WM * WN * 64);
-    qf_plan_note(ctx, 0x1000000ull | (unsigned long long)(BM << 8 | EPI << 2 | EXACT << 1 | (FUSED ? 1 : 0)),
+    if (guard.b_upper && !(BM == 64 && BN == 64 && EXACT && !EPI)) {
+        qf_set_error("k_zgemm: a right operand given by its upper tiles needs the exact 64 x 64 tiling (N=%d)", N);
+        return QF_ERR_STATE;
+    }
+    qf_plan_note(ctx, 0x1000000ull | (unsigned long long)(BM << 8 | (guard.b_upper ? 8 : 0) | EPI << 2 | EXACT << 1 | (FUSED ? 1 : 0)),
                  "{\"kernel\": \"k_zgemm<%d,%d%s>\", \"arithmetic\": \"fp64 3M, v_mfma_f64_16x16x4_f64\", \"tile\": [%d, %d], "
-                 "\"tiles\": %d, \"tile_share\": 1.0, \"workgroups\": %d, \"threads\": %d, \"exact_tiling\": %s, \"step_end\": \"%s\"}",
+                 "\"tiles\": %d, \"tile_share\": 1.0, \"workgroups\": %d, \"threads\": %d, \"exact_tiling\": %s, \"step_end\": \"%s\", "
+                 "\"right_operand\": \"%s\"}",
                  BM, BN, EPI ? ",EPI" : "", BM, BN, tiles_m * tiles_n, tiles_m * tiles_n, WM * WN * 64, EXACT ? "true" : "false",
-                 !EPI ? "none" : FUSED ? "fused (last tile decides)" : "two-kernel");
+                 !EPI ? "none" : FUSED ? "fused (last tile decides)" : "two-kernel",
+                 guard.b_upper ? "skew-Hermitian, upper tiles only" : "whole");
     hipLaunchKernelGGL((k_zgemm<BM, BN, WM, WN, EPI, EXACT, FUSED>), grid, block, smem, ctx->stream, N, tiles_m,
                        tiles_n, A, B, C, ep, guard);
     QF_HIP(hipGetLastError());
@@ -1397,6 +1547,21 @@
     return (N + c.BN - 1) / c.BN;
 }
 
+bool qf_gemm_b_upper_ok(int N)
+{
+    return N % 64 == 0 && pick_gemm(N).BM == 64;
+}
+
+int qf_launch_zgemm_b_upper(qf_ctx *ctx, const cplx *A, const cplx *B, cplx *C, qf_guard guard)
+{
+    if (ctx->N % 64 != 0) {
+        qf_set_error("qf_launch_zgemm_b_upper: N %% 64 == 0 only (N=%d)", ctx->N);
+        return QF_ERR_INVALID;
+    }
+    guard.b_upper = 1;
+    return launch<64, 64, 2, 2>(ctx, A, B, C, nullptr, guard);
+}
+
 int qf_launch_zgemm_tri(qf_ctx *ctx, const cplx *A, const cplx *B, const qf_epilogue *ep, qf_guard guard)
 {
     const int N = ctx->N;
@@ -1404,8 +1569,9 @@
         qf_set_error("qf_launch_zgemm_tri: not available for this context (N=%d)", N);
         return QF_ERR_STATE;
     }
-    static qf_smem_attr attr;
+    static qf_smem_attr attr, attr_up;
     QF_TRY(qf_smem_attr_set(attr, (const void *)k_zgemm_tri, ctx->device, TRI_SMEM_BYTES));
+    QF_TRY(qf_smem_attr_set(attr_up, (const void *)k_zgemm_tri_up, ctx->device, TRI_SMEM_BYTES));
     const int nt = N / 64;
     int E = ep->fused ? ctx->sk_epi_units_fused : ctx->sk_epi_units;
     if (E < -8) E = -8;
@@ -1434,12 +1600,16 @@
         sk.spin_limit = 1u << 14;
         ctx->debug_drop = 0;
     }
-    qf_plan_note(ctx, 0x2000000ull | (unsigned long long)(grid << 8 | (E & 0x3f) << 1 | (ep->fused ? 1 : 0)),
+    qf_plan_note(ctx, 0x2000000ull | (unsigned long long)(grid << 8 | (E & 0x3f) << 2 | (ep->whalf_upper_only ? 2 : 0) | (ep->fused ? 1 : 0)),
                  "{\"kernel\": \"k_zgemm_tri\", \"arithmetic\": \"fp64 3M, v_mfma_f64_16x16x4_f64\", \"tile\": [64, 64], \"tiles\": %d, "
                  "\"tile_share\": %.6f, \"workgroups\": %d, \"threads\": 256, \"partition\": \"stream-K over (tile, K-tile) units, "
-                 "contiguous ranges, epilogue weight E = %d K-tiles\", \"step_end\": \"%s\"}",
-                 sk.n_tiles, (double)sk.n_tiles / ((double)nt * nt), grid, E, ep->fused ? "fused (last finisher decides)" : "two-kernel");
-    hipLaunchKernelGGL(k_zgemm_tri, dim3(grid), dim3(256), TRI_SMEM_BYTES, ctx->stream, N, nt, (int)units, E, A, B, *ep, guard, sk);
+                 "contiguous ranges, epilogue weight E = %d K-tiles\", \"step_end\": \"%s\", \"whalf\": \"%s\"}",
+                 sk.n_tiles, (double)sk.n_tiles / ((double)nt * nt), grid, E, ep->fused ? "fused (last finisher decides)" : "two-kernel",
+                 ep->whalf_upper_only ? "upper tiles only (k_zgemm_tri_up)" : "mirrored");
+    if (ep->whalf_upper_only)
+        hipLaunchKernelGGL(k_zgemm_tri_up, dim3(grid), dim3(256), TRI_SMEM_BYTES, ctx->stream, N, nt, (int)units, E, A, B, *ep, guard, sk);
+    else
+        hipLaunchKernelGGL(k_zgemm_tri, dim3(grid), dim3(256), TRI_SMEM_BYTES, ctx->stream, N, nt, (int)units, E, A, B, *ep, guard, sk);
     QF_HIP(hipGetLastError());
     return QF_OK;
 }
```

Result: no change. 2700, median of 6 (+0.5%).
